# microsoft/StemGNN

Hardware: AMD Instinct MI355X
Metric: forecast-steps/sec (train) (higher is better)
Workload: dtype f32

## Files before the change

### include/stemgnn_hip.h

```cpp
#ifndef STEMGNN_HIP_H
#define STEMGNN_HIP_H

#include <stddef.h>
#include <stdint.h>

#ifdef __cplusplus
extern "C" {
#endif

#define SG_EINVAL (-10001)

#define SG_BLOCK_NPARAMS 33

const char* stemgnn_version(void);
int stemgnn_num_cus(void);

size_t stemgnn_table_floats(int W, int multi);
size_t stemgnn_packed_floats(int W, int multi);
size_t stemgnn_saved_floats(int B, int N, int W, int multi);
size_t stemgnn_scratch_floats(int B, int N, int W, int multi);
size_t stemgnn_gradpart_floats(int W, int multi, int nsplit);
size_t stemgnn_attn_saved_floats(int B, int N);
size_t stemgnn_attn_scratch_floats(int B, int N, int nchunk);
size_t stemgnn_scratch_offset_dG(int B, int N, int W, int multi);

int stemgnn_make_tables_host(int W, int multi, float* tables_host);

int stemgnn_attn_laplacian_fwd(const float* h, const float* wk, const float* wq, float alpha,
                               float drop_p, int training, const uint64_t* seed,
                               int B, int N, float* saved, float* attention_out, float* mul_L,
                               int parts, void* stream);
int stemgnn_attn_laplacian_bwd(const float* dL, const float* h, const float* wk, const float* wq,
                               float alpha, float drop_p, int training, const uint64_t* seed,
                               int B, int N, const float* saved, float* scratch, int nchunk,
                               float* dh, float* dwk, float* dwq, int parts, void* stream);
int stemgnn_attn_laplacian_bwd_ext(const float* dL, const float* dA_ext, const float* h, const float* wk, const float* wq,
                                   float alpha, float drop_p, int training, const uint64_t* seed,
                                   int B, int N, const float* saved, float* scratch, int nchunk,
                                   float* dh, float* dwk, float* dwq, int parts, void* stream);
int stemgnn_dropout_mask(float drop_p, const uint64_t* seed, int B, int N, float* mask, void* stream);
int stemgnn_dropout_seed_next(uint64_t* seed, uint64_t* used, void* stream);

int stemgnn_cheb_fwd(float* mul_L, int N, void* stream);
int stemgnn_cheb_bwd(const float* mul_L, const float* dmul_L, float* dL, float* scratch, int N, void* stream);

size_t stemgnn_eigh_scratch_floats(int N);
int stemgnn_eigh_fwd(float* mul_L, float* lam, float* U, float* scratch, int N, int nsweeps, void* stream);
int stemgnn_eigh_batched(float* mul_L, float* lam, float* U, float* scratch, int N, int batch, void* stream);
int stemgnn_eigh_status(void);
int stemgnn_eigh_cluster_fixes(void);

size_t stemgnn_split_planes_floats(int N, int K, int splits);
int stemgnn_split_weights_bf16(const float* B, int N, int K, int splits, void* planes, void* stream);
int stemgnn_glu_gemm_bf16(const float* A, const void* planes, float* C, int M, int N, int K, int splits, void* stream);
int stemgnn_glu_gemm_f32(const float* A, const float* B, float* C, int M, int N, int K, void* stream);

int stemgnn_sgemm_f32(const float* A, int lda, int a_kcontig, const float* B, int ldb, int b_kcontig, float* C, int ldc,
                      int M, int N, int K, int accumulate, void* stream);
int stemgnn_glu_combine_fwd(const float* U, const float* V, const float* bl, const float* br, float* out, float* gate,
                            float* lin, int M, int C, void* stream);
int stemgnn_glu_combine_bwd(const float* dout, const float* lin, const float* gate, float* dU, float* dV, int M, int C,
                            void* stream);
int stemgnn_colsum(const float* X, int M, int C, float* out, void* stream);

size_t stemgnn_gru_reserve_floats(int B, int S, int Hd);
size_t stemgnn_gru_fwd_scratch_floats(int B, int S, int Hd);
size_t stemgnn_gru_bwd_scratch_floats(int B, int S, int Hd, int W);
int stemgnn_gru_bwd_cus(int B, int Hd);
#define SG_GRU_PATH_WORDS 16
#define SG_GRU_FWD_FAMILY   0
#define SG_GRU_FWD_P        1
#define SG_GRU_FWD_K        2
#define SG_GRU_GI_STREAM    3
#define SG_GRU_BWD_FAMILY   4
#define SG_GRU_BWD_P        5
#define SG_GRU_BWD_KU       6
#define SG_GRU_BWD_SLICES   7
#define SG_GRU_IH_FOLDED    8
#define SG_GRU_HH_FORM      9
#define SG_GRU_IH_SLABS     10
#define SG_GRU_RANK2_OK     11
#define SG_GRU_WIDE_PASSES  12
#define SG_GRU_WIDE_MT      13
#define SG_GRU_WIDE_GWF     14
#define SG_GRU_WIDE_GWB     15
#define SG_GRU_FAM_STREAM   0
#define SG_GRU_FAM_CLUSTER1 1
#define SG_GRU_FAM_CLUSTER2 2
#define SG_GRU_FAM_CLUSTER4 3
#define SG_GRU_FAM_WIDE     4
#define SG_GRU_HH_SLABS     0
#define SG_GRU_HH_TILES     1
#define SG_GRU_HH_FLAT      2
int stemgnn_gru_paths(int B, int S, int Hd, int W, int cus, int* out );
int stemgnn_gru_fwd(const float* x, const float* w_ih, const float* w_hh, const float* b_ih, const float* b_hh,
                    int B, int S, int Hd, int W, float* scratch, float* h_ext, float* reserve, int* status,
                    void* stream);
int stemgnn_gru_bwd(const float* dh_all, const float* x, const float* w_hh, const float* h_ext,
                    const float* reserve, int B, int S, int Hd, int W, float* scratch,
                    float* dw_ih, float* dw_hh, float* db_ih, float* db_hh, int* status, void* stream);

int stemgnn_keyquery_wgrad(const float* h, const float* attn_scratch, float* dwk, float* dwq, int B, int N, void* stream);
int stemgnn_attn_dquery_reduce(float* attn_scratch, int B, int N, int nchunk, float* out, void* stream);
int stemgnn_keyquery_wgrad2(const float* h, const float* dkey, const float* dquery, float* dwk, float* dwq, int B, int N,
                            void* stream);
int stemgnn_gru_bwd_rank2_ok(int B, int Hd);
int stemgnn_gru_bwd_rank2(const float* dkey, const float* dquery, const float* wk, const float* wq, const float* x,
                          const float* w_hh, const float* h_ext, const float* reserve, int B, int S, int Hd, int W,
                          float* scratch, float* dw_ih, float* dw_hh, float* db_ih, float* db_hh, int* status, void* stream);
int stemgnn_gru_bwd_rank2_dq(const float* dkey, float* dquery, int nchunk, int flags, const float* wk, const float* wq, const float* x,
                             const float* w_hh, const float* h_ext, const float* reserve, int B, int S, int Hd, int W,
                             float* scratch, float* dw_ih, float* dw_hh, float* db_ih, float* db_hh, int* status, void* stream);
int stemgnn_gru_bwd_overlap_ok(int B, int S, int Hd, int W);
size_t stemgnn_gru_bwd_ctl_words(int S);
int stemgnn_gru_bwd_rank2_begin(const float* dkey, const float* dquery, const float* wk, const float* wq, const float* x,
                                const float* w_hh, const float* h_ext, const float* reserve, int B, int S, int Hd, int W,
                                float* scratch, float* dw_ih, float* dw_hh, float* db_ih, float* db_hh, int* status,
                                unsigned* ctl, void* stream);
int stemgnn_gru_bwd_rank2_finish(const float* dkey, const float* dquery, const float* wk, const float* wq, const float* x,
                                 const float* w_hh, const float* h_ext, const float* reserve, int B, int S, int Hd, int W,
                                 float* scratch, float* dw_ih, float* dw_hh, float* db_ih, float* db_hh, int* status,
                                 unsigned* ctl, void* side_stream, void* stream);
int stemgnn_gru_bwd_recur(const float* dh_all, const float* x, const float* w_hh, const float* h_ext, const float* reserve,
                          int B, int S, int Hd, int W, float* scratch, int* status, void* stream);
int stemgnn_gru_bwd_rank2_recur(const float* dkey, float* dquery, int nchunk, const float* wk, const float* wq, const float* x,
                                const float* w_hh, const float* h_ext, const float* reserve, int B, int S, int Hd, int W,
                                float* scratch, int* status, void* stream);
int stemgnn_gru_input_grad(const float* scratch, const float* w_ih, int B, int S, int Hd, int W, float* dx, void* stream);

int stemgnn_block_pack(const float* const* params_host, const float* tables, float* packed,
                       int W, int multi, void* stream);
int stemgnn_block_pack_panels(const float* const* params_host, const float* tables, float* packed, int W, int multi,
                              void* stream);
int stemgnn_glu_fused_repack(float* packed, int W, int multi, void* stream);
int stemgnn_block_unpack_grads(const float* gradpart, int nsplit, const float* tables,
                               float* const* grads_host, int W, int multi, int has_backcast, void* stream);

int stemgnn_gft_fwd(const float* mul_L, const float* X, long xs_b, long xs_n, long xs_t,
                    float* G, int B, int N, int W, void* stream);
int stemgnn_gft_bwd(const float* mul_L, const float* X, long xs_b, long xs_n, long xs_t,
                    const float* dG, float* dX, float* dmul_L, int accumulate,
                    int B, int N, int W, void* stream);
int stemgnn_gft_bwd_dt2(const float* X0, long xs0_b, long xs0_n, long xs0_t, const float* dG0, const float* X1, long xs1_b,
                        long xs1_n, long xs1_t, const float* dG1, float* dmul_L, int B, int N, int W, void* stream);

int stemgnn_spectral_glu_fwd(const float* packed, float* saved, int B, int N, int W, int multi, void* stream);
int stemgnn_spectral_glu_bwd(const float* packed, const float* saved, float* scratch, float* gradpart,
                             int nsplit, int parts, int B, int N, int W, int multi, void* stream);
size_t stemgnn_glu_split_floats(int W, int multi, int splits);
int stemgnn_glu_split_panels(const float* packed, float* split, int W, int multi, int splits, void* stream);
int stemgnn_spectral_glu_fwd_split(const float* packed, const float* split, float* saved, int B, int N, int W, int multi,
                                   int splits, void* stream);
size_t stemgnn_glu_warm_saved_floats(int W, int multi);
int stemgnn_spectral_glu_fwd_warm(const float* packed, const float* split, float* saved, int B, int N, int W, int multi,
                                  int splits, void* stream);
int stemgnn_spectral_glu_dgrad_split(const float* packed, const float* split, const float* saved, float* scratch,
                                     int B, int N, int W, int multi, int splits, void* stream);
int stemgnn_glu_fused_bf16_ok(int W, int multi, int splits);

int stemgnn_igft_heads_fwd(const float* const* params_host, const float* packed, float* saved,
                           const float* X, long xs_b, long xs_n, long xs_t,
                           float* forecast, int accumulate, float* backcast,
                           int B, int N, int W, int multi, void* stream);
int stemgnn_igft_heads_bwd(const float* const* params_host, const float* packed, const float* saved,
                           const float* X, long xs_b, long xs_n, long xs_t,
                           const float* dforecast, const float* dbackcast, const float* backcast,
                           float* scratch, float* gradpart, int nsplit, int parts,
                           int B, int N, int W, int multi, void* stream);

int stemgnn_shortcut_dx(const float* scratch, const float* bs_w, float* dX, int B, int N, int W, int multi, void* stream);

int stemgnn_block_wgrad(const float* const* params_host, const float* packed, const float* saved,
                        const float* X, long xs_b, long xs_n, long xs_t, const float* dforecast, int has_bc,
                        float* scratch, float* gradpart, int nsplit, int cu_percent,
                        int B, int N, int W, int multi, void* stream);
int stemgnn_block_wgrad_split(const float* const* params_host, const float* packed, const float* saved,
                              const float* X, long xs_b, long xs_n, long xs_t, const float* dforecast, int has_bc,
                              float* scratch, float* gradpart, int nsplit, int cu_percent, int B, int N, int W,
                              int multi, int splits, void* stream);

#define SG_PATH_GLU_FWD_FUSED   1
#define SG_PATH_GLU_DGRAD_FUSED 2
#define SG_PATH_HEADS_FWD_FUSED 4
#define SG_PATH_HEADS_BWD_FUSED 8
#define SG_PATH_HEADS_BWD_16W   16
#define SG_PATH_LONG_K          32
#define SG_PATH_WGRAD_FUSED     64
#define SG_PATH_GLU_WGRAD_FUSED 128
int stemgnn_block_paths(int B, int N, int W, int multi, int splits);

size_t stemgnn_infer_workspace_floats(int B, int N, int W, int multi);
size_t stemgnn_infer_workspace_split_floats(int B, int N, int W, int multi, int splits);
int stemgnn_gru_fwd_infer(const float* x, const float* w_ih, const float* w_hh, const float* b_ih, const float* b_hh,
                          int B, int S, int Hd, int W, float* scratch, float* h_ext, int* status, void* stream);
int stemgnn_spectral_glu_fwd_infer(const float* packed, float* ws, size_t ws_floats, int B, int N, int W, int multi,
                                   void* stream);
int stemgnn_spectral_glu_fwd_split_infer(const float* packed, const float* split, float* ws, size_t ws_floats, int B, int N,
                                         int W, int multi, int splits, void* stream);
int stemgnn_igft_heads_fwd_infer(const float* const* params_host, const float* packed, float* ws, size_t ws_floats,
                                 const float* X, long xs_b, long xs_n, long xs_t, float* forecast, int accumulate,
                                 float* backcast, int B, int N, int W, int multi, void* stream);

int stemgnn_fc_tail_supported(int W, int H);
size_t stemgnn_fc_tail_scratch_floats(int B, int N, int W, int H);
int stemgnn_fc_tail_fwd(const float* fsum, const float* w0, const float* b0, const float* w2, const float* b2,
                        int B, int N, int W, int H, float* forecast, void* stream);
int stemgnn_fc_tail_bwd(const float* dforecast, const float* fsum, const float* w0, const float* b0, const float* w2,
                        int B, int N, int W, int H, float* scratch, float* dfsum, float* dw0, float* db0,
                        float* dw2, float* db2, void* stream);
size_t stemgnn_fc_tail_train_scratch_floats(int B, int N, int W, int H);
int stemgnn_fc_tail_train(const float* fsum, const float* target, const float* w0, const float* b0, const float* w2,
                          const float* b2, int B, int N, int W, int H, float* scratch, float* forecast,
                          float* loss, double* loss_accum, float* dfsum, float* dw0, float* db0, float* dw2,
                          float* db2, void* stream);
int stemgnn_fc_tail_train_rows(const float* fsum, const float* target, const float* w0, const float* b0, const float* w2,
                               const float* b2, int B, int N, int W, int H, float* scratch, float* forecast, float* dfsum,
                               void* stream);
// ... 63 lines not shown
```

### stemgnn_amd/_lib.py

```python
import ctypes
import os
from ctypes import POINTER, c_char_p, c_float, c_int, c_long, c_size_t, c_void_p

_HERE = os.path.dirname(os.path.abspath(__file__))
LIB_PATH = os.environ.get("STEMGNN_HIP_LIB", os.path.join(_HERE, "libstemgnn_hip.so"))
SG_BLOCK_NPARAMS = 33
SG_EINVAL = -10001
SG_LOSS = {"mse": 0, "mae": 1, "huber": 2}
SG_PATH = {"glu_fwd_fused": 1, "glu_dgrad_fused": 2, "heads_fwd_fused": 4, "heads_bwd_fused": 8, "heads_bwd_16w": 16,
           "long_k": 32, "wgrad_fused": 64, "glu_wgrad_fused": 128}
SG_GRU_PATH_WORDS = 16
SG_GRU_WORD = {"fwd_family": 0, "fwd_P": 1, "fwd_K": 2, "gi_stream": 3, "bwd_family": 4, "bwd_P": 5, "bwd_KU": 6,
               "bwd_slices": 7, "ih_folded": 8, "hh_form": 9, "ih_slabs": 10, "rank2_ok": 11, "wide_passes": 12,
               "wide_MT": 13, "wide_GWf": 14, "wide_GWb": 15}
SG_GRU_FAM = {"stream": 0, "cluster1": 1, "cluster2": 2, "cluster4": 3, "wide": 4}
SG_GRU_HH = {"slabs": 0, "tiles": 1, "flat": 2}


def gru_paths(B, S, Hd, W, cus=0):
    out = (c_int * SG_GRU_PATH_WORDS)()
    check(load().stemgnn_gru_paths(B, S, Hd, W, cus, out), "stemgnn_gru_paths")
    return {k: int(out[i]) for k, i in SG_GRU_WORD.items()}


_P = c_void_p
_PP = POINTER(c_void_p)

SIGNATURES = {
    "stemgnn_version": (c_char_p, []),
    "stemgnn_num_cus": (c_int, []),
    "stemgnn_table_floats": (c_size_t, [c_int, c_int]),
    "stemgnn_packed_floats": (c_size_t, [c_int, c_int]),
    "stemgnn_saved_floats": (c_size_t, [c_int, c_int, c_int, c_int]),
    "stemgnn_scratch_floats": (c_size_t, [c_int, c_int, c_int, c_int]),
    "stemgnn_scratch_offset_dG": (c_size_t, [c_int, c_int, c_int, c_int]),
    "stemgnn_gradpart_floats": (c_size_t, [c_int, c_int, c_int]),
    "stemgnn_attn_saved_floats": (c_size_t, [c_int, c_int]),
    "stemgnn_attn_scratch_floats": (c_size_t, [c_int, c_int, c_int]),
    "stemgnn_make_tables_host": (c_int, [c_int, c_int, _P]),
    "stemgnn_attn_laplacian_fwd": (c_int, [_P, _P, _P, c_float, c_float, c_int, _P, c_int, c_int, _P, _P, _P, c_int, _P]),
    "stemgnn_attn_laplacian_bwd": (c_int, [_P, _P, _P, _P, c_float, c_float, c_int, _P, c_int, c_int, _P, _P, c_int,
                                           _P, _P, _P, c_int, _P]),
    "stemgnn_attn_laplacian_bwd_ext": (c_int, [_P, _P, _P, _P, _P, c_float, c_float, c_int, _P, c_int, c_int, _P, _P, c_int,
                                               _P, _P, _P, c_int, _P]),
    "stemgnn_dropout_mask": (c_int, [c_float, _P, c_int, c_int, _P, _P]),
    "stemgnn_dropout_seed_next": (c_int, [_P, _P, _P]),
    "stemgnn_cheb_fwd": (c_int, [_P, c_int, _P]),
    "stemgnn_cheb_bwd": (c_int, [_P, _P, _P, _P, c_int, _P]),
    "stemgnn_eigh_scratch_floats": (c_size_t, [c_int]),
    "stemgnn_eigh_fwd": (c_int, [_P, _P, _P, _P, c_int, c_int, _P]),
    "stemgnn_eigh_batched": (c_int, [_P, _P, _P, _P, c_int, c_int, _P]),
    "stemgnn_eigh_status": (c_int, []),
    "stemgnn_eigh_cluster_fixes": (c_int, []),
    "stemgnn_split_planes_floats": (c_size_t, [c_int, c_int, c_int]),
    "stemgnn_split_weights_bf16": (c_int, [_P, c_int, c_int, c_int, _P, _P]),
    "stemgnn_glu_gemm_bf16": (c_int, [_P, _P, _P, c_int, c_int, c_int, c_int, _P]),
    "stemgnn_glu_gemm_f32": (c_int, [_P, _P, _P, c_int, c_int, c_int, _P]),
    "stemgnn_sgemm_f32": (c_int, [_P, c_int, c_int, _P, c_int, c_int, _P, c_int, c_int, c_int, c_int, c_int, _P]),
    "stemgnn_glu_combine_fwd": (c_int, [_P, _P, _P, _P, _P, _P, _P, c_int, c_int, _P]),
    "stemgnn_glu_combine_bwd": (c_int, [_P, _P, _P, _P, _P, c_int, c_int, _P]),
    "stemgnn_colsum": (c_int, [_P, c_int, c_int, _P, _P]),
    "stemgnn_glu_fused_repack": (c_int, [_P, c_int, c_int, _P]),
    "stemgnn_shortcut_dx": (c_int, [_P, _P, _P, c_int, c_int, c_int, c_int, _P]),
    "stemgnn_gru_reserve_floats": (c_size_t, [c_int, c_int, c_int]),
    "stemgnn_gru_fwd_scratch_floats": (c_size_t, [c_int, c_int, c_int]),
    "stemgnn_gru_bwd_scratch_floats": (c_size_t, [c_int, c_int, c_int, c_int]),
    "stemgnn_gru_bwd_cus": (c_int, [c_int, c_int]),
    "stemgnn_gru_paths": (c_int, [c_int, c_int, c_int, c_int, c_int, POINTER(c_int)]),
    "stemgnn_gru_fwd": (c_int, [_P, _P, _P, _P, _P, c_int, c_int, c_int, c_int, _P, _P, _P, _P, _P]),
    "stemgnn_gru_bwd": (c_int, [_P, _P, _P, _P, _P, c_int, c_int, c_int, c_int, _P, _P, _P, _P, _P, _P, _P]),
    "stemgnn_gru_bwd_rank2_ok": (c_int, [c_int, c_int]),
    "stemgnn_gru_bwd_rank2": (c_int, [_P, _P, _P, _P, _P, _P, _P, _P, c_int, c_int, c_int, c_int, _P, _P, _P, _P, _P, _P, _P]),
    "stemgnn_gru_bwd_rank2_dq": (c_int, [_P, _P, c_int, c_int, _P, _P, _P, _P, _P, _P, c_int, c_int, c_int, c_int, _P, _P, _P, _P, _P, _P, _P]),
    "stemgnn_gru_bwd_overlap_ok": (c_int, [c_int, c_int, c_int, c_int]),
    "stemgnn_gru_bwd_ctl_words": (c_size_t, [c_int]),
    "stemgnn_gru_bwd_rank2_begin": (c_int, [_P, _P, _P, _P, _P, _P, _P, _P, c_int, c_int, c_int, c_int, _P, _P, _P, _P, _P, _P, _P, _P]),
    "stemgnn_gru_bwd_rank2_finish": (c_int, [_P, _P, _P, _P, _P, _P, _P, _P, c_int, c_int, c_int, c_int, _P, _P, _P, _P, _P, _P, _P, _P, _P]),
    "stemgnn_gru_bwd_recur": (c_int, [_P, _P, _P, _P, _P, c_int, c_int, c_int, c_int, _P, _P, _P]),
    "stemgnn_gru_bwd_rank2_recur": (c_int, [_P, _P, c_int, _P, _P, _P, _P, _P, _P, c_int, c_int, c_int, c_int, _P, _P, _P]),
    "stemgnn_gru_input_grad": (c_int, [_P, _P, c_int, c_int, c_int, c_int, _P, _P]),
    "stemgnn_keyquery_wgrad": (c_int, [_P, _P, _P, _P, c_int, c_int, _P]),
    "stemgnn_attn_dquery_reduce": (c_int, [_P, c_int, c_int, c_int, _P, _P]),
    "stemgnn_keyquery_wgrad2": (c_int, [_P, _P, _P, _P, _P, c_int, c_int, _P]),
    "stemgnn_fc_tail_supported": (c_int, [c_int, c_int]),
    "stemgnn_fc_tail_scratch_floats": (c_size_t, [c_int, c_int, c_int, c_int]),
    "stemgnn_fc_tail_fwd": (c_int, [_P, _P, _P, _P, _P, c_int, c_int, c_int, c_int, _P, _P]),
    "stemgnn_fc_tail_bwd": (c_int, [_P, _P, _P, _P, _P, c_int, c_int, c_int, c_int, _P, _P, _P, _P, _P, _P, _P]),
    "stemgnn_fill_zero": (c_int, [_P, c_size_t, _P]),
    "stemgnn_rmsprop_step": (c_int, [_P, _P, _P, c_size_t, _P, c_float, c_float, c_int, c_float, _P]),
    "stemgnn_adam_step": (c_int, [_P, _P, _P, _P, c_size_t, _P, _P, c_float, c_float, c_float, c_int, c_float, _P]),
    "stemgnn_grad_norm_partials": (c_size_t, [c_size_t]),
    "stemgnn_grad_sqsum": (c_int, [_P, c_size_t, c_float, _P, _P]),
    "stemgnn_rmsprop_step_ext": (c_int, [_P, _P, _P, c_size_t, _P, c_float, c_float, c_int, c_float, c_float, c_float, c_int,
                                         _P, _P, _P]),
    "stemgnn_adam_step_ext": (c_int, [_P, _P, _P, _P, c_size_t, _P, _P, c_float, c_float, c_float, c_int, c_float, c_float,
                                      c_int, c_float, c_int, _P, _P, _P]),
    "stemgnn_normalize_series": (c_int, [_P, _P, _P, c_int, _P, c_long, c_int, _P]),
    "stemgnn_window_gather": (c_int, [_P, _P, _P, _P, c_int, c_int, c_int, c_int, c_long, _P, _P]),
    "stemgnn_window_gather_queue": (c_int, [_P, _P, _P, _P, _P, c_int, c_int, c_int, c_int, c_long, _P, _P]),
    "stemgnn_window_gather_pair": (c_int, [_P, _P, _P, _P, _P, c_int, c_int, c_int, c_int, c_long, _P, _P]),
    "stemgnn_window_gather_queue_pair": (c_int, [_P, _P, _P, _P, _P, _P, c_int, c_int, c_int, c_int, c_long, _P, _P]),
    "stemgnn_mse_scratch_floats": (c_size_t, []),
    "stemgnn_mse_fwd": (c_int, [_P, _P, c_size_t, _P, _P, _P, _P]),
    "stemgnn_mse_bwd": (c_int, [_P, _P, c_size_t, _P, _P, _P]),
    "stemgnn_roll_window": (c_int, [_P, _P, _P, _P, c_int, c_int, c_int, c_int, c_int, c_int, _P]),
    "stemgnn_forecast_store": (c_int, [_P, _P, _P, _P, _P, c_int, c_int, c_int, c_long, _P]),
    "stemgnn_eval_scratch_doubles": (c_size_t, [c_long, c_int, c_int]),
    "stemgnn_eval_out_doubles": (c_size_t, [c_int, c_int]),
    "stemgnn_eval_metrics": (c_int, [_P, _P, _P, _P, c_long, c_int, c_int, _P, _P, _P]),
    "stemgnn_eval_scratch_doubles_masked": (c_size_t, [c_long, c_int, c_int]),
    "stemgnn_eval_metrics_masked": (c_int, [_P, _P, _P, _P, c_long, c_int, c_int, _P, _P, _P]),
    "stemgnn_block_pack": (c_int, [_PP, _P, _P, c_int, c_int, _P]),
    "stemgnn_block_pack_panels": (c_int, [_PP, _P, _P, c_int, c_int, _P]),
    "stemgnn_block_unpack_grads": (c_int, [_P, c_int, _P, _PP, c_int, c_int, c_int, _P]),
    "stemgnn_gft_fwd": (c_int, [_P, _P, c_long, c_long, c_long, _P, c_int, c_int, c_int, _P]),
    "stemgnn_gft_bwd": (c_int, [_P, _P, c_long, c_long, c_long, _P, _P, _P, c_int, c_int, c_int, c_int, _P]),
    "stemgnn_gft_bwd_dt2": (c_int, [_P, c_long, c_long, c_long, _P, _P, c_long, c_long, c_long, _P, _P, c_int, c_int, c_int, _P]),
    "stemgnn_spectral_glu_fwd": (c_int, [_P, _P, c_int, c_int, c_int, c_int, _P]),
    "stemgnn_spectral_glu_bwd": (c_int, [_P, _P, _P, _P, c_int, c_int, c_int, c_int, c_int, c_int, _P]),
    "stemgnn_glu_split_floats": (c_size_t, [c_int, c_int, c_int]),
    "stemgnn_glu_split_panels": (c_int, [_P, _P, c_int, c_int, c_int, _P]),
    "stemgnn_glu_fused_bf16_ok": (c_int, [c_int, c_int, c_int]),
    "stemgnn_block_paths": (c_int, [c_int, c_int, c_int, c_int, c_int]),
    "stemgnn_spectral_glu_fwd_split": (c_int, [_P, _P, _P, c_int, c_int, c_int, c_int, c_int, _P]),
    "stemgnn_glu_warm_saved_floats": (c_size_t, [c_int, c_int]),
    "stemgnn_spectral_glu_fwd_warm": (c_int, [_P, _P, _P, c_int, c_int, c_int, c_int, c_int, _P]),
    "stemgnn_spectral_glu_dgrad_split": (c_int, [_P, _P, _P, _P, c_int, c_int, c_int, c_int, c_int, _P]),
    "stemgnn_igft_heads_fwd": (c_int, [_PP, _P, _P, _P, c_long, c_long, c_long, _P, c_int, _P,
                                       c_int, c_int, c_int, c_int, _P]),
    "stemgnn_igft_heads_bwd": (c_int, [_PP, _P, _P, _P, c_long, c_long, c_long, _P, _P, _P, _P, _P, c_int, c_int,
                                       c_int, c_int, c_int, c_int, _P]),
    "stemgnn_fc_tail_train_scratch_floats": (c_size_t, [c_int, c_int, c_int, c_int]),
    "stemgnn_fc_tail_train": (c_int, [_P, _P, _P, _P, _P, _P, c_int, c_int, c_int, c_int, _P, _P, _P, _P, _P, _P, _P, _P,
                                      _P, _P]),
    "stemgnn_fc_tail_train_rows": (c_int, [_P, _P, _P, _P, _P, _P, c_int, c_int, c_int, c_int, _P, _P, _P, _P]),
    "stemgnn_fc_tail_train_finish": (c_int, [_P, c_int, c_int, c_int, c_int, _P, _P, _P, _P, _P, _P, _P]),
    "stemgnn_target_valid_count": (c_int, [_P, c_size_t, _P, _P]),
    "stemgnn_fc_tail_train_loss": (c_int, [_P, _P, _P, _P, _P, _P, c_int, c_int, c_int, c_int, c_int, c_float, _P, _P, _P, _P,
                                           _P, _P, _P, _P, _P, _P, _P]),
    "stemgnn_fc_tail_train_rows_loss": (c_int, [_P, _P, _P, _P, _P, _P, c_int, c_int, c_int, c_int, c_int, c_float, _P, _P, _P,
                                                _P, _P]),
    "stemgnn_fc_tail_train_finish_loss": (c_int, [_P, c_int, c_int, c_int, c_int, _P, _P, _P, _P, _P, _P, _P, _P]),
    "stemgnn_infer_workspace_floats": (c_size_t, [c_int, c_int, c_int, c_int]),
    "stemgnn_infer_workspace_split_floats": (c_size_t, [c_int, c_int, c_int, c_int, c_int]),
    "stemgnn_gru_fwd_infer": (c_int, [_P, _P, _P, _P, _P, c_int, c_int, c_int, c_int, _P, _P, _P, _P]),
    "stemgnn_spectral_glu_fwd_infer": (c_int, [_P, _P, c_size_t, c_int, c_int, c_int, c_int, _P]),
    "stemgnn_spectral_glu_fwd_split_infer": (c_int, [_P, _P, _P, c_size_t, c_int, c_int, c_int, c_int, c_int, _P]),
    "stemgnn_igft_heads_fwd_infer": (c_int, [_PP, _P, _P, c_size_t, _P, c_long, c_long, c_long, _P, c_int, _P,
                                             c_int, c_int, c_int, c_int, _P]),
    "stemgnn_block_wgrad": (c_int, [_PP, _P, _P, _P, c_long, c_long, c_long, _P, c_int, _P, _P, c_int, c_int,
                                    c_int, c_int, c_int, c_int, _P]),
    "stemgnn_block_wgrad_split": (c_int, [_PP, _P, _P, _P, c_long, c_long, c_long, _P, c_int, _P, _P, c_int, c_int,
                                          c_int, c_int, c_int, c_int, c_int, _P]),
}

_lib = None


class StemGNNHipError(RuntimeError):
    pass


def load():
    global _lib
    if _lib is not None:
        return _lib
    if not os.path.isfile(LIB_PATH):
        raise StemGNNHipError(
            f"{LIB_PATH} not found -- build it with `python __graft_entry__.py` (hipcc --offload-arch=gfx950); "
            "stemgnn_amd has no CPU / eager fallback.")
    lib = ctypes.CDLL(LIB_PATH)
    for name, (res, args) in SIGNATURES.items():
        fn = getattr(lib, name)
        fn.restype = res
        fn.argtypes = args
    _lib = lib
    return lib


def check(rc, what):
    if rc != 0:
        if rc == SG_EINVAL:
            raise StemGNNHipError(f"{what}: invalid argument (SG_EINVAL)")
        raise StemGNNHipError(f"{what}: HIP error {-rc}")


def ptr_array(tensors):
    arr = (c_void_p * SG_BLOCK_NPARAMS)()
    for i, t in enumerate(tensors):
        arr[i] = None if t is None else t.data_ptr()
    return arr
```

### stemgnn_amd/base_model.py

```python
import itertools
import os

import torch
import torch.nn as nn

from . import _lib, ops
from .ops import FcTail, FcTailMse, GruFront, SpectralHotPath, StockBlockFn

_instance_counter = itertools.count()
_BLOCK_FIELDS = ("forecast", "forecast_result", "backcast", "backcast_short_cut")
_FC_TAIL_MAX_W, _FC_TAIL_MAX_H = 64, 32


class GLU(nn.Module):

    def __init__(self, input_channel, output_channel):
        super().__init__()
        self.linear_left = nn.Linear(input_channel, output_channel)
        self.linear_right = nn.Linear(input_channel, output_channel)

    def forward(self, x):
        if not x.is_cuda:
            raise _lib.StemGNNHipError(f"input is on {x.device}: stemgnn_amd.GLU runs only on a HIP device (no CPU fallback)")
        lead = x.shape[:-1]
        out = ops.GluFn.apply(x.reshape(-1, x.shape[-1]), self.linear_left.weight, self.linear_left.bias,
                              self.linear_right.weight, self.linear_right.bias)
        return out.reshape(*lead, out.shape[-1])


class StockBlockLayer(nn.Module):

    def __init__(self, time_step, unit, multi_layer, stack_cnt=0):
        super().__init__()
        self.time_step, self.unit, self.multi, self.stack_cnt = time_step, unit, multi_layer, stack_cnt
        wide = time_step * multi_layer
        self.weight = nn.Parameter(torch.empty(1, 4, 1, wide, wide))
        nn.init.xavier_normal_(self.weight)
        self.forecast = nn.Linear(wide, wide)
        self.forecast_result = nn.Linear(wide, time_step)
        if stack_cnt == 0:
            self.backcast = nn.Linear(wide, time_step)
        self.backcast_short_cut = nn.Linear(time_step, time_step)
        self.output_channel = 4 * multi_layer
        glu_out = time_step * self.output_channel
        self.GLUs = nn.ModuleList(
            GLU(time_step * 4 if layer == 0 else glu_out, glu_out) for layer in range(3) for _branch in range(2))

    def hip_params(self):
        out = [self.weight]
        for name in _BLOCK_FIELDS:
            lin = getattr(self, name, None)
            out += [None, None] if lin is None else [lin.weight, lin.bias]
        for g in self.GLUs:
            out += [g.linear_left.weight, g.linear_left.bias, g.linear_right.weight, g.linear_right.bias]
        return out

    def forward(self, x, mul_L):
        if not x.is_cuda:
            raise _lib.StemGNNHipError(
                f"input is on {x.device}: stemgnn_amd.StockBlockLayer runs only on a HIP device (no CPU fallback)")
        B, _, N, W = x.shape
        forecast, backcast = StockBlockFn.apply(x.reshape(B, N, W), mul_L, self.multi, self.stack_cnt == 0,
                                                *self.hip_params())
        return forecast, (backcast.unsqueeze(1) if backcast is not None else None)


class Model(nn.Module):
    def __init__(self, units, stack_cnt, time_step, multi_layer, horizon=1, dropout_rate=0.5, leaky_rate=0.2,
                 device='cpu'):
        super().__init__()
        self.unit, self.stack_cnt, self.alpha = units, stack_cnt, leaky_rate
        self.time_step, self.horizon, self.multi_layer = time_step, horizon, multi_layer
        if time_step > _FC_TAIL_MAX_W or horizon > _FC_TAIL_MAX_H:
            raise _lib.StemGNNHipError(
                f"Model(time_step={time_step}, horizon={horizon}): the fc tail kernels (csrc/tail.hip) cover time_step <= "
                f"{_FC_TAIL_MAX_W} and horizon <= {_FC_TAIL_MAX_H}; stemgnn_amd has no torch fallback for larger ones")
        self.dropout_rate = float(dropout_rate)
        self.weight_key = nn.Parameter(torch.zeros(units, 1))
        nn.init.xavier_uniform_(self.weight_key.data, gain=1.414)
        self.weight_query = nn.Parameter(torch.zeros(units, 1))
        nn.init.xavier_uniform_(self.weight_query.data, gain=1.414)
        self.GRU = nn.GRU(time_step, units)
        self.stock_block = nn.ModuleList(
            StockBlockLayer(time_step, units, multi_layer, stack_cnt=i) for i in range(stack_cnt))
        self.fc = nn.Sequential(nn.Linear(time_step, time_step), nn.LeakyReLU(), nn.Linear(time_step, horizon))
        self._seed = None
        self._instance = next(_instance_counter)
        self.hot_state = ops.HotPathState()
        self.to(device)

    def _next_seed(self, device):
        if self._seed is None or self._seed.device != device:
            rank = 0
            if torch.distributed.is_available() and torch.distributed.is_initialized():
                rank = torch.distributed.get_rank()
            key = (torch.cuda.default_generators[device.index if device.index is not None
                                                 else torch.cuda.current_device()].initial_seed()
                   + 0x9E3779B97F4A7C15 * (self._instance + 1) + 0xD1B54A32D192ED03 * rank) % (1 << 62)
            self._seed = torch.tensor([key, 0], dtype=torch.int64, device=device)
        used = torch.empty_like(self._seed)
        _lib.check(_lib.load().stemgnn_dropout_seed_next(self._seed.data_ptr(), used.data_ptr(),
                                                         torch.cuda.current_stream(device).cuda_stream), "dropout_seed_next")
        return used

    def set_dropout_seed(self, seed, offset=0, device=None):
        device = device or self.weight_key.device
        self._seed = torch.tensor([int(seed), int(offset)], dtype=torch.int64, device=device)

    def __getstate__(self):
        state = self.__dict__.copy()
        state["_seed"] = None
        state["hot_state"] = None
        return state

    def __setstate__(self, state):
        self.__dict__.update(state)
        self._instance = next(_instance_counter)
        self.hot_state = ops.HotPathState()

    def train(self, mode=True):
        out = super().train(mode)
        dev = self.weight_key.device if hasattr(self, "weight_key") else None
        if dev is not None and dev.type == "cuda" and ops.gru_status_exists(dev) \
                and not torch.cuda.is_current_stream_capturing():
            ops.check_gru_status(dev)
            if os.environ.get("STEMGNN_SPECTRAL", "cheb") == "eig":
                ops.check_eigh_status(dev)
        return out

    def prefetch_side(self, device=None, batch=None):
        hs = self.hot_state
        if not hs.overlap or hs.prepacked is not None:
            return
        device = device or self.weight_key.device
        blocks = (self.stock_block[0].hip_params(), self.stock_block[1].hip_params())
        ops.prepack_blocks(hs, blocks, self.time_step, self.multi_layer, device,
                           batch_shape=None if batch is None else (int(batch), self.unit))
        if self.training and self.dropout_rate > 0.0:
            with torch.cuda.stream(ops._side_stream(device)):
                hs.preseed = self._next_seed(device)

    def hot_path(self, x):
        if not x.is_cuda:
            raise _lib.StemGNNHipError(
                f"input is on {x.device}: stemgnn_amd.Model runs only on a HIP device (no CPU fallback)")
        if self.stack_cnt > 2:
            raise AttributeError("'NoneType' object has no attribute 'unsqueeze'")
        if self.stack_cnt < 2:
            raise IndexError("list index out of range")
        x = x.contiguous()
        blocks = (self.stock_block[0].hip_params(), self.stock_block[1].hip_params())
        use_drop = self.training and self.dropout_rate > 0.0
        hs = self.hot_state
        if hs.overlap and hs.prepacked is None:
            self.prefetch_side(x.device, batch=x.shape[0])
        seed, hs.preseed = hs.preseed, None
        if seed is not None and not torch.cuda.is_current_stream_capturing():
            seed.record_stream(torch.cuda.current_stream())
        if os.environ.get("STEMGNN_GRU", "hip") == "miopen":
            h, _ = self.GRU(x.permute(2, 0, 1).contiguous())
        else:
            g = self.GRU
            h = GruFront.apply(x, g.weight_ih_l0, g.weight_hh_l0, g.bias_ih_l0, g.bias_hh_l0, hs)
            hs.gru_front_live = True
        if use_drop and seed is None:
            seed = self._next_seed(x.device)
        params = blocks[0] + blocks[1]
        return SpectralHotPath.apply(h, x, self.weight_key, self.weight_query, self.multi_layer, self.alpha,
                                     self.dropout_rate, self.training, seed, hs, *params)

    def loss(self, x, target, loss_out=None, accum=None, unit_grad=False, return_attention=False, *, kind="mse",
             huber_delta=1.0, ignore_nan=False):
        if kind not in _lib.SG_LOSS:
            raise ValueError(f"unknown loss kind {kind!r}: one of {sorted(_lib.SG_LOSS)}")
        self._require_fc_tail()
        fsum, attention, _ = self.hot_path(x)
        loss = FcTailMse.apply(fsum, target, self.fc[0].weight, self.fc[0].bias, self.fc[2].weight, self.fc[2].bias,
                               self.hot_state, loss_out, accum, bool(unit_grad) and torch.is_grad_enabled(), kind,
                               float(huber_delta) if kind == "huber" else 0.0, bool(ignore_nan))
        return (loss, attention) if return_attention else loss

    def _require_fc_tail(self):
        if not _lib.load().stemgnn_fc_tail_supported(self.time_step, self.horizon):
            raise _lib.StemGNNHipError(f"fc tail: time_step={self.time_step}, horizon={self.horizon} outside the HIP kernels' "
                                       "range (time_step <= 64, horizon <= 32); stemgnn_amd has no torch fallback")

    def predict(self, x):
        self._require_fc_tail()
        if not x.is_cuda:
            raise _lib.StemGNNHipError(
                f"input is on {x.device}: stemgnn_amd.Model runs only on a HIP device (no CPU fallback)")
        if self.stack_cnt > 2:
            raise AttributeError("'NoneType' object has no attribute 'unsqueeze'")
        if self.stack_cnt < 2:
            raise IndexError("list index out of range")
        g = self.GRU
        blocks = self.stock_block[0].hip_params() + self.stock_block[1].hip_params()
        with torch.no_grad():
            return ops.forecast_forward(x, (g.weight_ih_l0, g.weight_hh_l0, g.bias_ih_l0, g.bias_hh_l0), self.weight_key,
                                        self.weight_query, self.multi_layer, self.alpha, self.dropout_rate, blocks,
                                        (self.fc[0].weight, self.fc[0].bias, self.fc[2].weight, self.fc[2].bias))

    def forward(self, x):
        self._require_fc_tail()
        fsum, attention, _ = self.hot_path(x)
        return FcTail.apply(fsum, self.fc[0].weight, self.fc[0].bias, self.fc[2].weight, self.fc[2].bias,
                            self.hot_state), attention
```

### stemgnn_amd/csrc/glu_fused.h

```cpp
#pragma once
#include <hip/hip_runtime.h>
#include <stdint.h>

#include <type_traits>

#include "gemm2.h"
#include "layout.h"

constexpr int GF_NI = 4;
#ifndef GF_PF
#define GF_PF 2
#endif
#ifndef GF_ABL
#define GF_ABL 0
#endif

__device__ __forceinline__ float gf_sigmoid(float v) { return __frcp_rn(1.f + __expf(-v)); }
#ifndef GF_NT_STORES
#define GF_NT_STORES 1
#endif
#if GF_NT_STORES
#define GF_ST(p, v) __builtin_nontemporal_store((v), (p))
#else
#define GF_ST(p, v) (*(p) = (v))
#endif

struct GfPackArgs {
  const float* wp[2][3];
  float* wf[2];
  int K[3], np[2][3], cp[2][3];
  GfGeom g;
};
static __global__ __launch_bounds__(256) void sg_pack_fused_kernel(const GfPackArgs a) {
  const int r = blockIdx.y;
  const size_t e = (size_t)blockIdx.x * 256 + threadIdx.x;
  if (e >= (size_t)a.g.ns * GF_STAGE) return;
  int s = (int)(e / GF_STAGE), l = 0;
  while (l < 2 && s >= a.g.nst[l]) { s -= a.g.nst[l]; ++l; }
  const int hp = 16 / a.g.rs[l], nc = 256 * hp;
  const int w = (int)(e % GF_STAGE);
  const int kk = w / nc, p = w % nc;
  const int wave = p / (64 * hp), rem = p % (64 * hp), h = rem >> 6, fi = (rem & 63) >> 1, t = rem & 1;
  const int c = wave * 32 * hp + h * 32 + fi, k = s * a.g.rs[l] + kk;
  float v = 0.f;
  if (k < a.K[l] && c < a.cp[r][l]) v = a.wp[r][l][(size_t)k * a.np[r][l] + ((c >> 4) << 5) + (c & 15) + 16 * t];
  a.wf[r][e] = v;
}

struct GfArgs {
  const float* G;
  const float* wf[2];
  const float* bias[2][3];
  float* out[2][3];
  float* gate[2][3];
  int cp[2][3];
  int nst[3];
  int KG, KP0, KA, M, nrb, ns;
};

template <int N>
__device__ __forceinline__ void gf_wait_vm() { asm volatile("s_waitcnt vmcnt(%0)" ::"n"(N) : "memory"); }

struct GfRing {
  const float* src;
  float* ring;
  int next, last, wbuf, wave, nstages;
  __device__ __forceinline__ void issue(int q) {
    __builtin_amdgcn_global_load_lds((const __attribute__((address_space(1))) void*)(src + q * 256),
                                     (__attribute__((address_space(3))) void*)(ring + wbuf * GF_STAGE + (wave * GF_NI + q) * 256),
                                     16, 0, 0);
  }
  __device__ __forceinline__ void advance() {
    if (next < last) src += GF_STAGE;
    ++next;
    wbuf = wbuf + 1 == nstages ? 0 : wbuf + 1;
  }
};

template <int MT>
struct GfTile {
  static constexpr int BM = 32 * MT, LDA = 32 * MT + 2;
  static constexpr int STAGES = MT == 3 ? 4 : 5;
  static __device__ __forceinline__ int row(int i, int reg, int lane) {
    return i < 2 ? 2 * g2_row_of(reg, lane) + i : 64 + g2_row_of(reg, lane);
  }
};
template <int MT, int HP>
__device__ __forceinline__ void gf_stage(const float* __restrict__ Aq, const float* __restrict__ A2,
                                         const float* __restrict__ Bs, sg_f32x16 (&acc)[MT][HP][2], GfRing& rg) {
  constexpr int NC = 256 * HP, RS = 16 / HP, STEPS = RS / 2, LDA = GfTile<MT>::LDA;
  constexpr int EVERY = STEPS / GF_NI;
  float2 fa[STEPS], fb[STEPS][HP];
  float fc[STEPS];
  auto rd = [&](int st) {
    fa[st] = *reinterpret_cast<const float2*>(Aq + 2 * st * LDA);
    if constexpr (MT == 3) fc[st] = A2[2 * st * LDA];
#pragma unroll
    for (int h = 0; h < HP; ++h) fb[st][h] = *reinterpret_cast<const float2*>(Bs + 2 * st * NC + h * 64);
  };
#pragma unroll
  for (int st = 0; st < GF_PF && st < STEPS; ++st) rd(st);
#pragma unroll
  for (int st = 0; st < STEPS; ++st) {
    float a[3];
    a[0] = fa[st].x; a[1] = fa[st].y; a[2] = MT == 3 ? fc[st] : 0.f;
    __builtin_amdgcn_sched_barrier(0);
    if (!(GF_ABL & 2)) acc[0][0][0] = __builtin_amdgcn_mfma_f32_32x32x2f32(a[0], fb[st][0].x, acc[0][0][0], 0, 0, 0);
    if (st + GF_PF < STEPS) rd(st + GF_PF);
    __builtin_amdgcn_sched_barrier(0);
    if (!(GF_ABL & 2)) acc[0][0][1] = __builtin_amdgcn_mfma_f32_32x32x2f32(a[0], fb[st][0].y, acc[0][0][1], 0, 0, 0);
    if (!(GF_ABL & 4) && st % EVERY == 0 && st / EVERY < GF_NI) rg.issue(st / EVERY);
    __builtin_amdgcn_sched_barrier(0);
    if (!(GF_ABL & 2)) {
#pragma unroll
      for (int i = 0; i < MT; ++i)
#pragma unroll
        for (int h = 0; h < HP; ++h) {
          if (i == 0 && h == 0) continue;
          acc[i][h][0] = __builtin_amdgcn_mfma_f32_32x32x2f32(a[i], fb[st][h].x, acc[i][h][0], 0, 0, 0);
          acc[i][h][1] = __builtin_amdgcn_mfma_f32_32x32x2f32(a[i], fb[st][h].y, acc[i][h][1], 0, 0, 0);
        }
    }
  }
}

template <int MT, int HP, bool LAST, bool INF = false>
__device__ __forceinline__ void gf_layer(float* As, GfRing& rg, int& rbuf, int nst, int lane, int wave,
                                         const float (&bl)[2], const float (&br)[2], float* __restrict__ outp,
                                         float* __restrict__ gatep, int cp, int M, int m0, int KA) {
// ... 63 lines not shown
              GF_ST(&po[(size_t)rl * cp], o[reg][i]);
              if constexpr (!INF) GF_ST(&pg[(size_t)rl * cp], gs[reg][i]);
            }
          }
      }
    }
  }
  if constexpr (!LAST) asm volatile("s_waitcnt lgkmcnt(0)" ::: "memory");
  if (GF_ABL & 1) {
    if (acc[0][0][0][0] + acc[MT - 1][HP - 1][1][7] == 1.2345e-30f) As[0] = 1.f;
  }
}

template <int MT, int HP01, int HP2, bool INF = false>
static __global__ __launch_bounds__(256, 1) void sg_glu_fused_fwd_kernel(const GfArgs g) {
  using T = GfTile<MT>;
  extern __shared__ __attribute__((aligned(16))) float gf_lds[];
  float* As = gf_lds;
  const int L = blockIdx.x, xcd = L & 7;
  const int r = (xcd >> 2) & 1, rb = (L >> 3) * 4 + (xcd & 3);
  if (rb >= g.nrb) return;
  const int tid = threadIdx.x, lane = tid & 63;
  const int wave = __builtin_amdgcn_readfirstlane(tid >> 6);
  const int fi = lane & 31;
  const int m0 = rb * T::BM, M = g.M;

  GfRing rg;
  rg.ring = gf_lds + (size_t)g.KA * T::LDA;
  rg.wave = wave;
  rg.nstages = T::STAGES;
  rg.src = g.wf[r] + (size_t)wave * GF_NI * 256 + lane * 4;
  rg.next = 0; rg.last = g.ns - 1; rg.wbuf = 0;
#pragma unroll
  for (int p = 0; p < T::STAGES - 1; ++p) {
#pragma unroll
    for (int q = 0; q < GF_NI; ++q) rg.issue(q);
    rg.advance();
  }
  float bl[3][2], br[3][2];
#pragma unroll
  for (int l = 0; l < 3; ++l) {
    const int hp = l < 2 ? HP01 : HP2;
#pragma unroll
    for (int h = 0; h < 2; ++h) {
      const int c = wave * 32 * hp + h * 32 + fi;
      const bool ok = h < hp && c < g.cp[r][l];
      const int q = ((c >> 4) << 5) + (c & 15);
      const float* b = g.bias[r][l];
      const float x = b[ok ? q : 0], y = b[ok ? q + 16 : 0];
      bl[l][h] = ok ? x : 0.f;
      br[l][h] = ok ? y : 0.f;
    }
  }
  {
    const int KG = g.KG;
    const float* Gp = g.G + (size_t)m0 * KG;
    const int nlive = (M - m0 < T::BM ? M - m0 : T::BM) * KG;
    for (int idx = tid; idx < T::BM * KG; idx += 256) {
      const int i = idx / KG, k = idx - i * KG;
      const float v = Gp[idx < nlive ? idx : 0];
      As[k * T::LDA + i] = idx < nlive ? v : 0.f;
    }
    for (int idx = tid; idx < (g.KP0 - KG) * T::BM; idx += 256) As[(KG + idx / T::BM) * T::LDA + (idx % T::BM)] = 0.f;
  }
#pragma unroll
  for (int l = 0; l < 3; ++l)
#pragma unroll
    for (int h = 0; h < 2; ++h) asm volatile("" : "+v"(bl[l][h]), "+v"(br[l][h]));
  asm volatile("s_waitcnt lgkmcnt(0)" ::: "memory");
  int rbuf = 0;
  gf_layer<MT, HP01, false, INF>(As, rg, rbuf, g.nst[0], lane, wave, bl[0], br[0], g.out[r][0], g.gate[r][0], g.cp[r][0], M, m0, g.KA);
  gf_layer<MT, HP01, false, INF>(As, rg, rbuf, g.nst[1], lane, wave, bl[1], br[1], g.out[r][1], g.gate[r][1], g.cp[r][1], M, m0, g.KA);
  gf_layer<MT, HP2, true, INF>(As, rg, rbuf, g.nst[2], lane, wave, bl[2], br[2], g.out[r][2], g.gate[r][2], g.cp[r][2], M, m0, g.KA);
  gf_wait_vm<0>();
}

struct GdPackArgs {
  const float* wp[2][3];
  float* wd[2];
  int np[2][3];
  int CP, KG;
  GdGeom g;
};
static __global__ __launch_bounds__(256) void sg_pack_dgrad_kernel(const GdPackArgs a) {
  const int r = blockIdx.y;
  const size_t e = (size_t)blockIdx.x * 256 + threadIdx.x;
  if (e >= (size_t)a.g.ns[r] * GF_STAGE) return;
  int s = (int)(e / GF_STAGE);
  const int nt = a.g.nt, rs = a.g.rs, nc = 128 * nt;
  const int wi = (int)(e % GF_STAGE);
  const int sAB = a.g.nstA[r] + a.g.nstB[0] + a.g.nstB[1];
  if (s >= sAB) {
    s -= sAB;
    int ph = 0;
    if (s >= a.g.nstC[0]) { s -= a.g.nstC[0]; ph = 1; }
    const int kk = wi >> 6, kin = wi & 63;
    const int k2 = s * 64 + kk;
    const int t = k2 & 1, wf = k2 >> 1, w2 = wf >> 5, f2 = wf & 31;
    const int c2 = w2 * 32 * nt + 32 * ph + f2;
    float v = 0.f;
    if (w2 < 4 && c2 < a.CP && kin < a.KG) v = a.wp[r][0][(size_t)kin * a.np[r][0] + ((c2 >> 4) << 5) + (c2 & 15) + 16 * t];
    a.wd[r][e] = v;
    return;
  }
  const int kk = wi / nc, p = wi % nc;
  int wave, fi, j;
  if (nt == 2) { wave = p >> 6; fi = (p & 63) >> 1; j = p & 1; }
  else { wave = p >> 5; fi = p & 31; j = 0; }
  const int c = wave * 32 * nt + 32 * j + fi;
  float v = 0.f;
  if (s < a.g.nstA[r]) {
    const int q = s * rs + kk;
    if (q < a.np[r][2] && c < a.CP) v = a.wp[r][2][(size_t)c * a.np[r][2] + q];
  } else {
    s -= a.g.nstA[r];
    int ph = 0;
    if (s >= a.g.nstB[0]) { s -= a.g.nstB[0]; ph = 1; }
    const int k2 = s * rs + kk;
    const int t = k2 & 1, wf = k2 >> 1, w2 = wf >> 5, f2 = wf & 31;
    const int c2 = w2 * 32 * nt + 32 * ph + f2;
    if (w2 < 4 && c2 < a.CP && c < a.CP) v = a.wp[r][1][(size_t)c * a.np[r][1] + ((c2 >> 4) << 5) + (c2 & 15) + 16 * t];
  }
  a.wd[r][e] = v;
}

struct GdArgs {
  const float* dact2[2];
  const float* wd[2];
  const float* out1[2];
  const float* gate1[2];
  const float* out0[2];
  const float* gate0[2];
  float* dact1[2];
  float* dact0[2];
  float* dG[2];
  int np2[2], nstA[2], ns[2];
  int nstB[2], nstC[2];
  int CP, KG, M, nrb, KA;
};

template <int MT>
struct GdTile {
  static constexpr int BM = 32 * MT, LDA = 32 * MT + 2;
  static constexpr int STAGES = MT == 3 ? 3 : 5;
};

template <int MT, int NT>
__device__ __forceinline__ void gd_stage(const float* __restrict__ Aq, const float* __restrict__ A2,
                                         const float* __restrict__ Bs, sg_f32x16 (&acc)[MT][NT], GfRing& rg) {
  constexpr int NC = 128 * NT, RS = 32 / NT, STEPS = RS / 2, LDA = GdTile<MT>::LDA;
  constexpr int EVERY = STEPS / GF_NI;
  float2 fa[STEPS];
  float fc[STEPS];
  float fb[STEPS][2];
  auto rd = [&](int st) {
    fa[st] = *reinterpret_cast<const float2*>(Aq + 2 * st * LDA);
    if constexpr (MT == 3) fc[st] = A2[2 * st * LDA];
    if constexpr (NT == 2) {
      const float2 b = *reinterpret_cast<const float2*>(Bs + 2 * st * NC);
      fb[st][0] = b.x; fb[st][1] = b.y;
    } else {
      fb[st][0] = Bs[2 * st * NC]; fb[st][1] = 0.f;
    }
  };
#pragma unroll
  for (int st = 0; st < GF_PF && st < STEPS; ++st) rd(st);
#pragma unroll
  for (int st = 0; st < STEPS; ++st) {
    float a[3];
    a[0] = fa[st].x; a[1] = fa[st].y; a[2] = MT == 3 ? fc[st] : 0.f;
    __builtin_amdgcn_sched_barrier(0);
    if (!(GF_ABL & 2)) acc[0][0] = __builtin_amdgcn_mfma_f32_32x32x2f32(a[0], fb[st][0], acc[0][0], 0, 0, 0);
    if (st + GF_PF < STEPS) rd(st + GF_PF);
    __builtin_amdgcn_sched_barrier(0);
    if (!(GF_ABL & 2)) acc[1][0] = __builtin_amdgcn_mfma_f32_32x32x2f32(a[1], fb[st][0], acc[1][0], 0, 0, 0);
    if (!(GF_ABL & 4) && st % EVERY == 0 && st / EVERY < GF_NI) rg.issue(st / EVERY);
    __builtin_amdgcn_sched_barrier(0);
    if (!(GF_ABL & 2)) {
      if constexpr (MT == 3) acc[2][0] = __builtin_amdgcn_mfma_f32_32x32x2f32(a[2], fb[st][0], acc[2][0], 0, 0, 0);
      if constexpr (NT == 2) {
#pragma unroll
        for (int i = 0; i < MT; ++i) acc[i][1] = __builtin_amdgcn_mfma_f32_32x32x2f32(a[i], fb[st][1], acc[i][1], 0, 0, 0);
      }
    }
  }
}

template <int MT>
__device__ __forceinline__ void gd_stage_c(const float* __restrict__ Aq, const float* __restrict__ A2,
                                           const float* __restrict__ Bs, sg_f32x16& acc, sg_f32x16& acc2, bool extra,
                                           GfRing& rg) {
  constexpr int STEPS = 32, EVERY = STEPS / GF_NI, PF = 4, LDA = GdTile<MT>::LDA;
  float fa[STEPS], fb[STEPS], fc[STEPS];
  auto rd = [&](int st) {
    fa[st] = Aq[2 * st * LDA];
    fb[st] = Bs[2 * st * 64];
    if constexpr (MT == 3) fc[st] = A2[2 * st * LDA];
  };
#pragma unroll
  for (int st = 0; st < PF; ++st) rd(st);
#pragma unroll
  for (int st = 0; st < STEPS; ++st) {
    __builtin_amdgcn_sched_barrier(0);
    if (!(GF_ABL & 2)) acc = __builtin_amdgcn_mfma_f32_32x32x2f32(fa[st], fb[st], acc, 0, 0, 0);
    if constexpr (MT == 3) {
      if (extra && !(GF_ABL & 2)) acc2 = __builtin_amdgcn_mfma_f32_32x32x2f32(fc[st], fb[st], acc2, 0, 0, 0);
// ... 263 lines not shown
```

### stemgnn_amd/csrc/gru.hip

```cpp
#include <hip/hip_runtime.h>

#include "../../include/stemgnn_hip.h"
#include "gemm2.h"
#include "wgrad.h"
#include "dq_reduce.h"
#include "gemm_core.h"
#include "gru_wide.h"

#define SG_TRY(e)                                \
  do {                                           \
    hipError_t _e = (e);                         \
    if (_e != hipSuccess) return -(int)_e;       \
  } while (0)

__device__ __forceinline__ float gru_sigmoid(float v) { return 1.f / (1.f + expf(-v)); }
__device__ __forceinline__ int gru_uniform(int v) { return __builtin_amdgcn_readfirstlane(v); }

struct GruGiOp {
  const float *x, *w_ih, *b_ih;
  float* gi;
  int B, S, Hd, W;
  unsigned *za, *zb;
  unsigned na, nb;
  __device__ bool setup(int, int& M, int& N, int& K0, int& K1) const {
    M = S * B; N = 3 * Hd; K0 = 0; K1 = W;
    if (na + nb) {
      const unsigned nwg = gridDim.x * gridDim.y, id = blockIdx.y * gridDim.x + blockIdx.x;
      const unsigned per = (na + nb + nwg - 1) / nwg, hi = min(na + nb, (id + 1) * per);
      for (unsigned i = id * per + threadIdx.x; i < hi; i += blockDim.x) {
        if (i < na) za[i] = 0u;
        else zb[i - na] = 0u;
      }
    }
    return true;
  }
  __device__ float a(int, int i, int k) const {
    const int s = i / B, b = i - s * B;
    return x[((size_t)b * W + k) * S + s];
  }
  __device__ float b(int, int k, int j) const { return w_ih[(size_t)j * W + k]; }
  __device__ void epi(int, int i, int j, float v) const { gi[(size_t)i * 3 * Hd + j] = v + b_ih[j]; }
};

struct GruDxOp {
  const float *dgi, *w_ih;
  float* dx;
  int B, S, Hd, W;
  __device__ bool setup(int, int& M, int& N, int& K0, int& K1) const {
    M = S * B; N = W; K0 = 0; K1 = 3 * Hd;
    return true;
  }
  __device__ float a(int, int i, int k) const {
    const int b = i / S, s = i - b * S;
    return dgi[((size_t)s * B + b) * 3 * Hd + k];
  }
  __device__ float b(int, int k, int j) const { return w_ih[(size_t)k * W + j]; }
  __device__ void epi(int, int i, int j, float v) const {
    const int b = i / S, s = i - b * S;
    dx[((size_t)b * W + j) * S + s] = v;
  }
};

constexpr int GI_RB = 16, GI_NT = 192;
template <int W>
__global__ __launch_bounds__(GI_NT) void gru_gi_stream_kernel(const float* __restrict__ x, const float* __restrict__ w_ih,
                                                              const float* __restrict__ b_ih, float* __restrict__ gi, int B,
                                                              int S, int Hd, unsigned* __restrict__ za,
                                                              unsigned* __restrict__ zb, unsigned na, unsigned nb) {
  __shared__ float xs[GI_RB][W];
  const int tid = threadIdx.x;
  const int M = S * B, H3 = 3 * Hd, ncg = H3 >> 2;
  const int i0 = blockIdx.x * GI_RB;
  const int cg = blockIdx.y * GI_NT + tid;
  const bool live = cg < ncg;
  const int cgc = live ? cg : ncg - 1;
  float wf[4 * W];
  {
    const float* wp = w_ih + (size_t)4 * cgc * W;
    if ((reinterpret_cast<uintptr_t>(w_ih) & 15) == 0) {
#pragma unroll
      for (int q = 0; q < W; ++q) {
        const float4 v = reinterpret_cast<const float4*>(wp)[q];
        wf[4 * q] = v.x; wf[4 * q + 1] = v.y; wf[4 * q + 2] = v.z; wf[4 * q + 3] = v.w;
      }
    } else {
#pragma unroll
      for (int q = 0; q < 4 * W; ++q) wf[q] = wp[q];
    }
  }
  float4 bias;
  bias.x = b_ih[4 * cgc]; bias.y = b_ih[4 * cgc + 1]; bias.z = b_ih[4 * cgc + 2]; bias.w = b_ih[4 * cgc + 3];
  for (int e = tid; e < GI_RB * W; e += GI_NT) {
    const int r = e / W, k = e - r * W;
    const int i = i0 + r < M ? i0 + r : M - 1;
    const int sI = i / B, b = i - sI * B;
    xs[r][k] = x[((size_t)b * W + k) * S + sI];
  }
  if (na + nb) {
    const unsigned nwg = gridDim.x * gridDim.y, id = blockIdx.y * gridDim.x + blockIdx.x;
    const unsigned per = (na + nb + nwg - 1) / nwg, hi = min(na + nb, (id + 1) * per);
    for (unsigned i = id * per + tid; i < hi; i += GI_NT) {
      if (i < na) za[i] = 0u;
      else zb[i - na] = 0u;
    }
  }
  __syncthreads();
#pragma unroll 4
  for (int r = 0; r < GI_RB; ++r) {
    float a0 = 0.f, a1 = 0.f, a2 = 0.f, a3 = 0.f;
#pragma unroll
    for (int k = 0; k < W; ++k) {
      const float xv = xs[r][k];
      a0 = fmaf(xv, wf[k], a0);
      a1 = fmaf(xv, wf[W + k], a1);
      a2 = fmaf(xv, wf[2 * W + k], a2);
      a3 = fmaf(xv, wf[3 * W + k], a3);
    }
    if (live && i0 + r < M)
      *reinterpret_cast<float4*>(gi + (size_t)(i0 + r) * H3 + 4 * cg) = make_float4(a0 + bias.x, a1 + bias.y, a2 + bias.z, a3 + bias.w);
  }
}

__global__ void gru_transpose_kernel(const float* __restrict__ w, float* __restrict__ wT, int rows, int cols) {
  __shared__ float t[32][33];
  const int tx = threadIdx.x & 31, ty = threadIdx.x >> 5;
  const int r0 = blockIdx.y * 32, c0 = blockIdx.x * 32;
  for (int r = ty; r < 32; r += 8)
    t[r][tx] = (r0 + r < rows && c0 + tx < cols) ? w[(size_t)(r0 + r) * cols + c0 + tx] : 0.f;
  __syncthreads();
  for (int r = ty; r < 32; r += 8)
    if (c0 + r < cols && r0 + tx < rows) wT[(size_t)(c0 + r) * rows + r0 + tx] = t[tx][r];
}

template <bool RS>
__global__ __launch_bounds__(1024) void gru_fwd_kernel(const float* __restrict__ gi, const float* __restrict__ w_hhT,
                                                       const float* __restrict__ b_hh, int B, int S, int Hd,
                                                       float* __restrict__ h_all, float* __restrict__ reserve) {
  extern __shared__ __attribute__((aligned(16))) float smem[];
  float* hs = smem;
  float* part = smem + Hd;
  const int b = blockIdx.x;
  const int tid = threadIdx.x, lane = tid & 63, wave = tid >> 6;
  const int nub = (Hd + 63) >> 6;
  const int ks = nub >= 16 ? 1 : 16 / nub;
  const int kchunk = (Hd + ks - 1) / ks;
  const int nwork = nub * ks;
  const int H3 = 3 * Hd;
  for (int i = tid; i < Hd; i += 1024) hs[i] = 0.f;
  __syncthreads();
  for (int s = 0; s < S; ++s) {
    for (int item = wave; item < nwork; item += 16) {
      const int ub = item % nub, kq = item / nub;
      const int unit = ub * 64 + lane;
      const int uc = unit < Hd ? unit : Hd - 1;
      const int k0 = kq * kchunk, k1 = min(Hd, k0 + kchunk);
      float a0 = 0.f, a1 = 0.f, a2 = 0.f;
      const float* wp = w_hhT + (size_t)k0 * H3 + uc;
#pragma unroll 8
      for (int k = k0; k < k1; ++k) {
        const float hv = hs[k];
        a0 = fmaf(wp[0], hv, a0);
        a1 = fmaf(wp[Hd], hv, a1);
        a2 = fmaf(wp[2 * Hd], hv, a2);
        wp += H3;
      }
      if (unit < Hd) {
        part[(kq * 3 + 0) * Hd + unit] = a0;
        part[(kq * 3 + 1) * Hd + unit] = a1;
        part[(kq * 3 + 2) * Hd + unit] = a2;
      }
    }
    __syncthreads();
    const size_t row = (size_t)s * B + b;
    for (int i = tid; i < Hd; i += 1024) {
      float g0 = b_hh[i], g1 = b_hh[Hd + i], g2 = b_hh[2 * Hd + i];
      for (int q = 0; q < ks; ++q) {
        g0 += part[(q * 3 + 0) * Hd + i];
        g1 += part[(q * 3 + 1) * Hd + i];
        g2 += part[(q * 3 + 2) * Hd + i];
      }
      const float* gip = gi + row * H3;
      const float r = gru_sigmoid(gip[i] + g0);
      const float z = gru_sigmoid(gip[Hd + i] + g1);
      const float n = tanhf(gip[2 * Hd + i] + r * g2);
      const float hn = (1.f - z) * n + z * hs[i];
      if constexpr (RS) {
        float* rs = reserve + row * 4 * Hd;
        rs[i] = r; rs[Hd + i] = z; rs[2 * Hd + i] = n; rs[3 * Hd + i] = g2;
      }
      h_all[row * Hd + i] = hn;
      hs[i] = hn;
    }
    __syncthreads();
  }
}

__global__ __launch_bounds__(1024) void gru_bwd_kernel(const float* __restrict__ dout, const float* __restrict__ w_hh,
                                                       const float* __restrict__ h_all, const float* __restrict__ reserve,
                                                       int B, int S, int Hd, float* __restrict__ dgi,
                                                       float* __restrict__ dghn) {
  extern __shared__ __attribute__((aligned(16))) float smem[];
  float* dgh = smem;
  float* dhz = smem + 3 * Hd;
// ... 661 lines not shown
  const int smax_ws = (int)(ws_floats / ((size_t)f.ntiles * WG_TILE_FLOATS));
  if (smax_ws >= 1) { f.form = SG_GRU_HH_TILES; f.smax = smax_ws > 32 ? 32 : smax_ws; }
  return f;
}
struct GruPlan {
  int fwd_family, PF, KF, gi_stream;
  int bwd_family, P, KU, slices, fold_ih, hh_form, ih_sum, rank2_ok;
  GruWide wide;
};
static GruPlan gru_plan(int B, int S, int Hd, int W, int limit) {
  GruPlan p{};
  const int P2 = gru_pick_P2(B, Hd, limit);
  if (gru_pick_wide(B, Hd, P2, limit, &p.wide) > 0) {
    p.fwd_family = p.bwd_family = SG_GRU_FAM_WIDE;
  } else if (P2 > 0) {
    p.fwd_family = SG_GRU_FAM_CLUSTER4;
    p.PF = P2;
    {
      const int want = 7, uw = (Hd + want - 1) / want;
      if (uw <= 40 && B * want <= limit) p.PF = want;
    }
    const int UF = (Hd + p.PF - 1) / p.PF;
    p.KF = UF <= 32 ? 32 : (UF <= 34 ? 34 : (UF <= 40 ? 40 : (UF <= 48 ? 48 : (UF <= 58 ? 58 : 64))));
    const bool v4 = P2 <= 4 || P2 == 6;
    p.bwd_family = v4 ? SG_GRU_FAM_CLUSTER4 : SG_GRU_FAM_CLUSTER2;
    p.P = P2;
    p.KU = gru_pick_KU(Hd, P2);
    if (P2 == 6 && p.KU < 58) p.KU = 58;
    p.slices = (P2 == 6 || P2 == 8) ? 2 : 1;
    p.fold_ih = v4 && W <= GRU4_WMAX;
    p.rank2_ok = v4;
  } else {
    const int P = gru_pick_P(B, Hd, limit);
    p.fwd_family = p.bwd_family = P > 0 ? SG_GRU_FAM_CLUSTER1 : SG_GRU_FAM_STREAM;
    p.PF = p.P = P;
  }
  p.gi_stream = gru_gi_stream_env() && p.fwd_family != SG_GRU_FAM_WIDE && W == 12 && (Hd & 3) == 0;
  p.ih_sum = p.fold_ih ? B : GRU_NSPLIT;
  {
    float* const base = reinterpret_cast<float*>((uintptr_t)256);
    WgGemm q[2];
    gru_hh_gemms(q, base, base + (size_t)3 * S * B * Hd, base, base, base, Hd);
    p.hh_form = gru_hh_form(q, Hd).form;
  }
  return p;
}
extern "C" int stemgnn_gru_paths(int B, int S, int Hd, int W, int cus, int* out) {
  if (B <= 0 || S <= 0 || Hd <= 0 || W <= 0 || !out) return SG_EINVAL;
  const GruPlan p = gru_plan(B, S, Hd, W, cus > 0 ? gru_limit_of_cus(cus) : gru_resident_limit());
  const bool wide = p.fwd_family == SG_GRU_FAM_WIDE;
  out[SG_GRU_FWD_FAMILY] = p.fwd_family; out[SG_GRU_FWD_P] = p.PF; out[SG_GRU_FWD_K] = p.KF;
  out[SG_GRU_GI_STREAM] = p.gi_stream;
  out[SG_GRU_BWD_FAMILY] = p.bwd_family; out[SG_GRU_BWD_P] = p.P; out[SG_GRU_BWD_KU] = p.KU;
  out[SG_GRU_BWD_SLICES] = p.slices; out[SG_GRU_IH_FOLDED] = p.fold_ih; out[SG_GRU_HH_FORM] = p.hh_form;
  out[SG_GRU_IH_SLABS] = p.ih_sum; out[SG_GRU_RANK2_OK] = p.rank2_ok;
  out[SG_GRU_WIDE_PASSES] = wide ? (B + GW_BP - 1) / GW_BP : 0;
  out[SG_GRU_WIDE_MT] = wide ? p.wide.MT : 0;
  out[SG_GRU_WIDE_GWF] = wide ? gru_wide_gwf_class(p.wide) : 0;
  out[SG_GRU_WIDE_GWB] = wide ? gru_wide_gwb_class(p.wide) : 0;
  return 0;
}

extern "C" size_t stemgnn_gru_fwd_scratch_floats(int B, int S, int Hd) {
  return (size_t)3 * Hd * Hd + (size_t)3 * S * B * Hd + gru_xbuf_floats(B, Hd) + 4;
}
static size_t gru_bwd_scratch_base(int B, int S, int Hd, int W) {
  return (size_t)4 * S * B * Hd + (size_t)GRU_NSPLIT * 3 * Hd * (Hd + 1) + (size_t)gru_ih_slabs(B) * 3 * Hd * (W + 1) +
         gru_xbuf_floats(B, Hd) + 4 + (size_t)B * Hd + 8 + 136;
}
constexpr size_t GRU_OVL_CLAIMS = 64 * 33;
static size_t gru_ovl_words(int S) { return (((size_t)S + 4 + GRU_OVL_CLAIMS + 64 + 8) + 3) & ~(size_t)3; }
extern "C" size_t stemgnn_gru_bwd_scratch_floats(int B, int S, int Hd, int W) {
  return ((gru_bwd_scratch_base(B, S, Hd, W) + 3) & ~(size_t)3) + gru_ovl_words(S);
}
extern "C" size_t stemgnn_gru_bwd_ctl_words(int S) { return S > 0 ? gru_ovl_words(S) + 64 : 0; }

extern "C" int stemgnn_gru_bwd_cus(int B, int Hd) {
  if (B <= 0 || Hd <= 0) return 0;
  const GruPlan pl = gru_plan(B, Hd, Hd, 1, gru_resident_limit());
  if (pl.bwd_family == SG_GRU_FAM_WIDE) return pl.wide.P;
  return B * (pl.P > 0 ? pl.P : 1);
}

template <bool RS>
static int gru_fwd_impl(const float* x, const float* w_ih, const float* w_hh, const float* b_ih, const float* b_hh, int B,
                        int S, int Hd, int W, float* scratch, float* h_ext, float* reserve, int* status, void* stream) {
  if (!x || !w_ih || !w_hh || !b_ih || !b_hh || !scratch || !h_ext || (RS && !reserve) || !status || B <= 0 || S <= 0 ||
      Hd <= 0 || W <= 0)
    return SG_EINVAL;
  hipStream_t st = (hipStream_t)stream;
  const GruPlan pl = gru_plan(B, S, Hd, W, gru_resident_limit());
  const bool use_wide = pl.fwd_family == SG_GRU_FAM_WIDE, use_c4 = pl.fwd_family == SG_GRU_FAM_CLUSTER4;
  float* h_all = h_ext + (size_t)B * Hd;
  float* w_hhT = scratch;
  float* gi = scratch + (size_t)3 * Hd * Hd;
  gru_u64* xbuf2 = (gru_u64*)(scratch + ((((size_t)3 * Hd * Hd + (size_t)3 * S * B * Hd) + 1) & ~(size_t)1));
  size_t zn0 = 0, zn1 = 0;
  if (use_c4) {
    zn0 = (size_t)B * Hd; zn1 = ((size_t)2 * B * Hd + (size_t)8 * B) * 2;
  } else {
    SG_TRY(sg_zero_async(h_ext, (size_t)B * Hd * sizeof(float), st));
  }
  if (pl.gi_stream && (reinterpret_cast<uintptr_t>(gi) & 15) == 0) {
    const int ncg = 3 * Hd / 4;
    hipLaunchKernelGGL(gru_gi_stream_kernel<12>, dim3((S * B + GI_RB - 1) / GI_RB, (ncg + GI_NT - 1) / GI_NT), dim3(GI_NT), 0,
                       st, x, w_ih, b_ih, gi, B, S, Hd, reinterpret_cast<unsigned*>(h_ext), reinterpret_cast<unsigned*>(xbuf2),
                       (unsigned)zn0, (unsigned)zn1);
    SG_TRY(hipGetLastError());
  } else {
    GruGiOp op{x, w_ih, b_ih, gi, B, S, Hd, W, reinterpret_cast<unsigned*>(h_ext), reinterpret_cast<unsigned*>(xbuf2),
               (unsigned)zn0, (unsigned)zn1};
    SG_TRY((sg_launch_gemm<GruGiOp, 64, 64, true, true, false>(op, S * B, 3 * Hd, 1, st)));
  }
  if (use_wide) {
    float* xb = scratch + ((((size_t)3 * Hd * Hd + (size_t)3 * S * B * Hd) + 3) & ~(size_t)3);
    SG_TRY(gru_wide_fwd<RS>(gi, w_hh, b_hh, B, S, Hd, pl.wide, xb, status, h_all, reserve, st));
    return 0;
  }
  if (use_c4) {
    gru_u64* xbuf = xbuf2;
    gru_u64* xid = xbuf + (size_t)2 * B * Hd;
    static const int allow_fast = !(getenv("STEMGNN_GRU_FAST_XCD") && atoi(getenv("STEMGNN_GRU_FAST_XCD")) == 0);
    const int PF = pl.PF, KF = pl.KF;
    const dim3 grid4(8 * ((B + 7) / 8) * PF);
#define GRU_F4K(PP, KK) hipLaunchKernelGGL((gru_fwd_cluster4_kernel<PP, KK, RS>), grid4, dim3((PP + 2) * 64), 0, st, gi, w_hh, \
                                           b_hh, B, S, Hd, xbuf, status, h_all, reserve, xid, allow_fast)
#define GRU_F4(PP) do { if (KF == 32) GRU_F4K(PP, 32); else if (KF == 34) GRU_F4K(PP, 34); else if (KF == 40) GRU_F4K(PP, 40); \
                        else if (KF == 48) GRU_F4K(PP, 48); else if (KF == 58) GRU_F4K(PP, 58); else GRU_F4K(PP, 64); } while (0)
    if (PF == 1) GRU_F4(1); else if (PF == 2) GRU_F4(2); else if (PF == 4) GRU_F4(4); else if (PF == 5) GRU_F4(5);
    else if (PF == 6) GRU_F4(6); else if (PF == 7) GRU_F4(7); else GRU_F4(8);
#undef GRU_F4
#undef GRU_F4K
    SG_TRY(hipGetLastError());
    return 0;
  }
  if (pl.fwd_family == SG_GRU_FAM_CLUSTER1) {
    const int P = pl.PF;
    const GruCluster c = gru_cluster_geom(Hd, P);
    gru_u64* xbuf = (gru_u64*)(scratch + ((((size_t)3 * Hd * Hd + (size_t)3 * S * B * Hd) + 1) & ~(size_t)1));
    if (P > 1) SG_TRY(sg_zero_async(xbuf, (size_t)2 * B * Hd * sizeof(gru_u64), st));
    const size_t lds = (size_t)(Hd + GRU_KC + c.ksf * 3 * c.U) * sizeof(float);
    const dim3 grid(8 * ((B + 7) / 8) * P);
    hipLaunchKernelGGL((gru_fwd_cluster_kernel<GRU_KC, RS>), grid, dim3(1024), lds, st, gi, w_hh, b_hh, B, S, Hd, P, xbuf,
                       status, h_all, reserve);
    SG_TRY(hipGetLastError());
    return 0;
  }
  hipLaunchKernelGGL(gru_transpose_kernel, dim3((Hd + 31) / 32, (3 * Hd + 31) / 32), dim3(256), 0, st, w_hh, w_hhT,
                     3 * Hd, Hd);
  SG_TRY(hipGetLastError());
  const int nub = (Hd + 63) / 64;
  const int ks = nub >= 16 ? 1 : 16 / nub;
  const size_t lds = (size_t)(Hd + ks * 3 * Hd) * sizeof(float);
  if (lds > 64 * 1024) return SG_EINVAL;
  hipLaunchKernelGGL(gru_fwd_kernel<RS>, dim3(B), dim3(1024), lds, st, gi, w_hhT, b_hh, B, S, Hd, h_all, reserve);
  SG_TRY(hipGetLastError());
  return 0;
}

extern "C" int stemgnn_gru_fwd(const float* x, const float* w_ih, const float* w_hh, const float* b_ih,
                               const float* b_hh, int B, int S, int Hd, int W, float* scratch, float* h_ext,
                               float* reserve, int* status, void* stream) {
  return gru_fwd_impl<true>(x, w_ih, w_hh, b_ih, b_hh, B, S, Hd, W, scratch, h_ext, reserve, status, stream);
}
extern "C" int stemgnn_gru_fwd_infer(const float* x, const float* w_ih, const float* w_hh, const float* b_ih,
                                     const float* b_hh, int B, int S, int Hd, int W, float* scratch, float* h_ext,
                                     int* status, void* stream) {
  return gru_fwd_impl<false>(x, w_ih, w_hh, b_ih, b_hh, B, S, Hd, W, scratch, h_ext, nullptr, status, stream);
}

static int gru_wgrad_rows(const float* dgi, const float* dghn, const float* h_ext, const float* x, float* p_hh, float* p_ih,
                          int B, int S, int Hd, int W, int row0, int rows, int slab0, int nsplit, hipStream_t st_hh,
                          hipStream_t st_ih, bool do_ih = true, bool do_hh = true) {
  const int chunk = ((rows + nsplit - 1) / nsplit + 15) & ~15;
  if (do_hh) {
    G2Args g;
    G2SlabEpi e;
    g.A[0] = dgi + (size_t)row0 * 3 * Hd;  g.lda[0] = 3 * Hd; g.M[0] = 2 * Hd;
    g.A[1] = dghn + (size_t)row0 * Hd;     g.lda[1] = Hd;     g.M[1] = Hd;
    for (int r = 0; r < 2; ++r) { g.B[r] = h_ext + (size_t)row0 * Hd; g.ldb[r] = Hd; g.N[r] = Hd + 1; g.K[r] = rows; }
    g.nsplit = nsplit; g.chunk = chunk; g.b_ones_col = Hd;
    e.part[0] = p_hh + (size_t)slab0 * 2 * Hd * (Hd + 1);
    e.part[1] = p_hh + (size_t)GRU_NSPLIT * 2 * Hd * (Hd + 1) + (size_t)slab0 * Hd * (Hd + 1);
    SG_TRY((g2_launch<G2SlabEpi, false, false>(g, e, 2, st_hh)));
  }
  if (!do_ih) return 0;
  GruWihGradOp o2{dgi, x, p_ih + (size_t)slab0 * 3 * Hd * (W + 1), B, S, Hd, W, nsplit, chunk, row0, rows};
  SG_TRY((sg_launch_gemm<GruWihGradOp, 64, 32, false, false, false, 64>(o2, 3 * Hd, W + 1, nsplit, st_ih)));
  return 0;
}
extern "C" int stemgnn_gru_bwd_rank2_ok(int B, int Hd) {
  if (B <= 0 || Hd <= 0) return 0;
  return gru_plan(B, Hd, Hd, 1, gru_resident_limit()).rank2_ok;
}
static int gru_bwd_impl(const float* dh_all, const float* dkey, const float* dquery, const float* wk, const float* wq,
                        const float* x, const float* w_hh, const float* h_ext, const float* reserve, int B, int S, int Hd,
                        int W, float* scratch, float* dw_ih, float* dw_hh, float* db_ih, float* db_hh, int* status,
                        void* stream, int stages = 3, void* side = nullptr, unsigned* ctl = nullptr, int dq_nchunk = 0,
                        int wg_split = 0, bool no_wgrad = false);
extern "C" int stemgnn_gru_bwd(const float* dh_all, const float* x, const float* w_hh, const float* h_ext,
                               const float* reserve, int B, int S, int Hd, int W, float* scratch, float* dw_ih,
                               float* dw_hh, float* db_ih, float* db_hh, int* status, void* stream) {
  if (!dh_all) return SG_EINVAL;
  return gru_bwd_impl(dh_all, nullptr, nullptr, nullptr, nullptr, x, w_hh, h_ext, reserve, B, S, Hd, W, scratch, dw_ih, dw_hh,
                      db_ih, db_hh, status, stream);
}
extern "C" int stemgnn_gru_bwd_rank2(const float* dkey, const float* dquery, const float* wk, const float* wq, const float* x,
                                     const float* w_hh, const float* h_ext, const float* reserve, int B, int S, int Hd, int W,
                                     float* scratch, float* dw_ih, float* dw_hh, float* db_ih, float* db_hh, int* status,
                                     void* stream) {
  if (!dkey || !dquery || !wk || !wq || !stemgnn_gru_bwd_rank2_ok(B, Hd)) return SG_EINVAL;
  return gru_bwd_impl(nullptr, dkey, dquery, wk, wq, x, w_hh, h_ext, reserve, B, S, Hd, W, scratch, dw_ih, dw_hh, db_ih, db_hh,
                      status, stream);
}
__global__ __launch_bounds__(256) void sg_gru_fill_dq_kernel(uint32_t* __restrict__ p, size_t n16, unsigned nfill,
                                                             const float* __restrict__ dqpart, float* __restrict__ dquery, int B,
                                                             int N, int nchunk) {
  if (blockIdx.x < nfill) {
    uint4* q = reinterpret_cast<uint4*>(p);
    for (size_t k = (size_t)blockIdx.x * 256 + threadIdx.x; k < n16; k += (size_t)nfill * 256) q[k] = make_uint4(0u, 0u, 0u, 0u);
    return;
  }
  const size_t idx = (size_t)(blockIdx.x - nfill) * 256 + threadIdx.x;
  if (idx < (size_t)B * N) sg_dquery_reduce_one(dqpart, dquery, N, nchunk, idx);
}
__global__ void sg_gru_dq_reduce_kernel(const float* __restrict__ dqpart, float* __restrict__ dquery, int B, int N, int nchunk) {
  const size_t idx = (size_t)blockIdx.x * blockDim.x + threadIdx.x;
  if (idx < (size_t)B * N) sg_dquery_reduce_one(dqpart, dquery, N, nchunk, idx);
}
extern "C" int stemgnn_gru_bwd_rank2_dq(const float* dkey, float* dquery, int nchunk, int flags, const float* wk, const float* wq,
                                        const float* x, const float* w_hh, const float* h_ext, const float* reserve, int B, int S,
                                        int Hd, int W, float* scratch, float* dw_ih, float* dw_hh, float* db_ih, float* db_hh,
                                        int* status, void* stream) {
  if (!dkey || !dquery || nchunk <= 0 || (flags & ~1) || !wk || !wq || !stemgnn_gru_bwd_rank2_ok(B, Hd)) return SG_EINVAL;
  return gru_bwd_impl(nullptr, dkey, dquery, wk, wq, x, w_hh, h_ext, reserve, B, S, Hd, W, scratch, dw_ih, dw_hh, db_ih, db_hh,
                      status, stream, 3, nullptr, nullptr, nchunk, flags & 1);
}
extern "C" int stemgnn_gru_bwd_recur(const float* dh_all, const float* x, const float* w_hh, const float* h_ext,
                                     const float* reserve, int B, int S, int Hd, int W, float* scratch, int* status,
                                     void* stream) {
  if (!dh_all) return SG_EINVAL;
  return gru_bwd_impl(dh_all, nullptr, nullptr, nullptr, nullptr, x, w_hh, h_ext, reserve, B, S, Hd, W, scratch, nullptr, nullptr,
                      nullptr, nullptr, status, stream, 3, nullptr, nullptr, 0, 0, true);
}
extern "C" int stemgnn_gru_bwd_rank2_recur(const float* dkey, float* dquery, int nchunk, const float* wk, const float* wq,
                                           const float* x, const float* w_hh, const float* h_ext, const float* reserve, int B,
// ... 262 lines not shown
```

### stemgnn_amd/csrc/pack.hip

```cpp
#include <hip/hip_runtime.h>
#include <math.h>

#include "../../include/stemgnn_hip.h"
#include "devattr.h"
#include "glu_fused.h"
#include "layout.h"

#define SG_TRY(e)                                \
  do {                                           \
    hipError_t _e = (e);                         \
    if (_e != hipSuccess) return -(int)_e;       \
  } while (0)

struct SgBlockParams { const float* p[SG_BLOCK_NPARAMS]; };
struct SgBlockGrads { float* p[SG_BLOCK_NPARAMS]; };

__host__ __device__ inline int sg_pidx_glu(int g, int side, int bias) { return 9 + 4 * g + 2 * side + bias; }

static void exact_cos_sin(long idx, long n, double* c, double* s) {
  idx %= n;
  if ((4 * idx) % n == 0) {
    static const double cs[4] = {1, 0, -1, 0}, sn[4] = {0, 1, 0, -1};
    const long qd = 4 * idx / n;
    *c = cs[qd]; *s = sn[qd];
    return;
  }
  const double ang = 2.0 * M_PI * (double)idx / (double)n;
  *c = cos(ang); *s = sin(ang);
}

extern "C" int stemgnn_make_tables_host(int W, int multi, float* t) {
  if (W <= 0 || multi <= 0 || !t) return SG_EINVAL;
  const SgDims d = sg_dims(1, 1, W, multi);
  const SgTableLayout L = sg_table_layout(d);
  for (int tt = 0; tt < W; ++tt)
    for (int f = 0; f < W; ++f) {
      double c, s;
      exact_cos_sin((long)tt * f, W, &c, &s);
      t[L.cosW + tt * W + f] = (float)c;
      t[L.sinW + tt * W + f] = (float)s;
    }
  const int Wm = d.Wm, h = Wm / 2;
  for (int f = 0; f < d.nf[0]; ++f) {
    const double cf = (f == 0 || (Wm % 2 == 0 && f == h)) ? 1.0 : 2.0;
    for (int tau = 0; tau < Wm; ++tau) {
      double c, s;
      exact_cos_sin((long)f * tau, Wm, &c, &s);
      t[L.cinvR + (size_t)f * Wm + tau] = (float)(cf * c / Wm);
    }
  }
  for (int fi = 0; fi < d.nf[1]; ++fi) {
    const int f = fi + 1;
    for (int tau = 0; tau < Wm; ++tau) {
      double c, s;
      exact_cos_sin((long)f * tau, Wm, &c, &s);
      t[L.cinvI + (size_t)fi * Wm + tau] = (float)(-2.0 * s / Wm);
    }
  }
  return 0;
}

extern "C" const char* stemgnn_version(void) { return "stemgnn_hip 0.1 gfx950"; }
extern "C" int stemgnn_num_cus(void) { return sg_num_cus(); }
extern "C" size_t stemgnn_table_floats(int W, int multi) { return sg_table_layout(sg_dims(1, 1, W, multi)).total; }
extern "C" size_t stemgnn_packed_floats(int W, int multi) { return sg_packed_layout(sg_dims(1, 1, W, multi)).total_ext; }
extern "C" size_t stemgnn_saved_floats(int B, int N, int W, int multi) { return sg_saved_layout(sg_dims(B, N, W, multi)).total; }
extern "C" size_t stemgnn_scratch_floats(int B, int N, int W, int multi) { return sg_scratch_layout(sg_dims(B, N, W, multi)).total; }
extern "C" size_t stemgnn_scratch_offset_dG(int B, int N, int W, int multi) { return sg_scratch_layout(sg_dims(B, N, W, multi)).dG; }
extern "C" size_t stemgnn_gradpart_floats(int W, int multi, int nsplit) {
  return sg_grad_layout(sg_dims(1, 1, W, multi), nsplit).total;
}

__global__ void sg_pack_kernel(SgBlockParams prm, const float* __restrict__ tab, float* __restrict__ packed, SgDims d,
                               SgPackedLayout P, SgTableLayout T) {
  const size_t idx = (size_t)blockIdx.x * blockDim.x + threadIdx.x;
  if (idx >= P.total) return;
  const int W = d.W, Wm = d.Wm, C = d.C;
  float val = 0.f;
  if (idx >= P.wfold) {
    const size_t e = idx - P.wfold;
    const int kk = (int)(e / d.WmP), o = (int)(e - (size_t)kk * d.WmP);
    const int r = kk >= d.CP2[0];
    const int c = kk - (r ? d.CP2[0] : 0);
    if (c < d.U[r] && o < Wm) {
      const int kq = c / d.nf[r], fi = c - kq * d.nf[r];
      const float* cinv = tab + (r ? T.cinvI : T.cinvR) + (size_t)fi * Wm;
      const float* wt = prm.p[0] + (size_t)kq * Wm * Wm + o;
      float s0 = 0.f, s1 = 0.f, s2 = 0.f, s3 = 0.f;
      int tau = 0;
      for (; tau + 3 < Wm; tau += 4) {
        s0 = fmaf(cinv[tau], wt[(size_t)tau * Wm], s0);
        s1 = fmaf(cinv[tau + 1], wt[(size_t)(tau + 1) * Wm], s1);
        s2 = fmaf(cinv[tau + 2], wt[(size_t)(tau + 2) * Wm], s2);
        s3 = fmaf(cinv[tau + 3], wt[(size_t)(tau + 3) * Wm], s3);
      }
      for (; tau < Wm; ++tau) s0 = fmaf(cinv[tau], wt[(size_t)tau * Wm], s0);
      val = (s0 + s1) + (s2 + s3);
    }
    packed[idx] = val;
    return;
  }
  for (int r = 0; r < 2; ++r)
    for (int l = 0; l < 3; ++l) {
      const int np = sg_glu_np(d, l, r), kin = sg_glu_kin(d, l), cu = sg_glu_cu(d, l, r);
      const int g = 2 * l + r;
      if (idx >= P.w[r][l] && idx < P.w[r][l] + (size_t)kin * np) {
        const size_t e = idx - P.w[r][l];
        const int kk = (int)(e / np), q = (int)(e - (size_t)kk * np);
        const int c = ((q >> 5) << 4) + (q & 15), side = (q >> 4) & 1;
        if (c < cu) {
          const int ch = l < 2 ? c : sg_l2_orig_channel(d, r, c);
          const float* w = prm.p[sg_pidx_glu(g, side, 0)];
          if (l == 0) {
            const int kq = kk / W + 1, t = kk - (kq - 1) * W;
            const float* row = w + (size_t)ch * (4 * W) + kq * W;
            const float* dt = tab + (r ? T.sinW : T.cosW) + t * W;
            float s = 0.f;
            for (int f = 0; f < W; ++f) s = fmaf(dt[f], row[f], s);
            val = r ? -s : s;
          } else if (kk < C) {
            val = w[(size_t)ch * C + kk];
          }
        }
        packed[idx] = val;
        return;
      }
      if (idx >= P.b[r][l] && idx < P.b[r][l] + (size_t)np) {
        const int q = (int)(idx - P.b[r][l]);
        const int c = ((q >> 5) << 4) + (q & 15), side = (q >> 4) & 1;
        if (c < cu) {
          const int ch = l < 2 ? c : sg_l2_orig_channel(d, r, c);
          val = prm.p[sg_pidx_glu(g, side, 1)][ch];
        }
        packed[idx] = val;
        return;
      }
    }
}

extern "C" int stemgnn_block_pack_panels(const float* const* params_host, const float* tables, float* packed, int W,
                                         int multi, void* stream) {
  if (!params_host || !tables || !packed || W <= 0 || multi <= 0) return SG_EINVAL;
  SgBlockParams prm;
  for (int i = 0; i < SG_BLOCK_NPARAMS; ++i) prm.p[i] = params_host[i];
  for (int i = 0; i < SG_BLOCK_NPARAMS; ++i)
    if (!prm.p[i] && i != 5 && i != 6) return SG_EINVAL;
  const SgDims d = sg_dims(1, 1, W, multi);
  const SgPackedLayout P = sg_packed_layout(d);
  const SgTableLayout T = sg_table_layout(d);
  const unsigned blocks = (unsigned)((P.total + 255) / 256);
  hipLaunchKernelGGL(sg_pack_kernel, dim3(blocks), dim3(256), 0, (hipStream_t)stream, prm, tables, packed, d, P, T);
  SG_TRY(hipGetLastError());
  return 0;
}
extern "C" int stemgnn_block_pack(const float* const* params_host, const float* tables, float* packed, int W,
                                  int multi, void* stream) {
  const int rc = stemgnn_block_pack_panels(params_host, tables, packed, W, multi, stream);
  if (rc) return rc;
  return stemgnn_glu_fused_repack(packed, W, multi, stream);
}

extern "C" int stemgnn_glu_fused_repack(float* packed, int W, int multi, void* stream) {
  if (!packed || W <= 0 || multi <= 0) return SG_EINVAL;
  const SgDims d = sg_dims(1, 1, W, multi);
  const SgPackedLayout P = sg_packed_layout(d);
  const GfGeom gg = gf_geom(d);
  if (gg.ok) {
    GfPackArgs a;
    a.g = gg;
    for (int l = 0; l < 3; ++l) {
      a.K[l] = sg_glu_kin(d, l);
      for (int r = 0; r < 2; ++r) {
        a.wp[r][l] = packed + P.w[r][l];
        a.np[r][l] = sg_glu_np(d, l, r);
        a.cp[r][l] = sg_glu_cp(d, l, r);
      }
    }
    for (int r = 0; r < 2; ++r) a.wf[r] = packed + P.wfused[r];
    const unsigned fb = (unsigned)(((size_t)gg.ns * GF_STAGE + 255) / 256);
    hipLaunchKernelGGL(sg_pack_fused_kernel, dim3(fb, 2), dim3(256), 0, (hipStream_t)stream, a);
    SG_TRY(hipGetLastError());
  }
  const GdGeom gd = gd_geom(d);
  if (gd.ok) {
    GdPackArgs a;
    a.g = gd;
    a.CP = d.CP; a.KG = d.KG;
    for (int l = 0; l < 3; ++l)
      for (int r = 0; r < 2; ++r) {
        a.wp[r][l] = packed + P.w[r][l];
        a.np[r][l] = sg_glu_np(d, l, r);
      }
    for (int r = 0; r < 2; ++r) a.wd[r] = packed + P.wdgrad[r];
    const int nsmax = gd.ns[0] > gd.ns[1] ? gd.ns[0] : gd.ns[1];
    const unsigned fb = (unsigned)(((size_t)nsmax * GF_STAGE + 255) / 256);
    hipLaunchKernelGGL(sg_pack_dgrad_kernel, dim3(fb, 2), dim3(256), 0, (hipStream_t)stream, a);
    SG_TRY(hipGetLastError());
  }
  return 0;
}

struct SgParamOffsets { size_t prefix[SG_BLOCK_NPARAMS + 1]; };

__global__ void sg_unpack_kernel(const float* __restrict__ part, const float* __restrict__ tab, SgBlockGrads gr,
                                 SgParamOffsets PO, SgDims d, SgGradLayout G, SgTableLayout T, int has_bc) {
  const size_t idx = (size_t)blockIdx.x * blockDim.x + threadIdx.x;
  if (idx >= PO.prefix[SG_BLOCK_NPARAMS]) return;
  int pi = 0;
  while (pi + 1 < SG_BLOCK_NPARAMS && idx >= PO.prefix[pi + 1]) ++pi;
  float* out = gr.p[pi];
  if (!out) return;
  const size_t e = idx - PO.prefix[pi];
  const int W = d.W, Wm = d.Wm, C = d.C;
  float val = 0.f;
  if (pi == 0) {
    const int kq = (int)(e / ((size_t)Wm * Wm));
    const int rem = (int)(e - (size_t)kq * Wm * Wm);
    const int tau = rem / Wm, o = rem - tau * Wm;
    const float* wf = part + G.wfold;
    float s0 = 0.f, s1 = 0.f;
#pragma unroll 4
    for (int f = 0; f < d.nf[0]; ++f)
      s0 = fmaf(tab[T.cinvR + (size_t)f * Wm + tau], wf[(size_t)(kq * d.nf[0] + f) * d.WmP + o], s0);
#pragma unroll 4
    for (int f = 0; f < d.nf[1]; ++f)
      s1 = fmaf(tab[T.cinvI + (size_t)f * Wm + tau], wf[(size_t)(d.CP2[0] + kq * d.nf[1] + f) * d.WmP + o], s1);
    val = s0 + s1;
  } else if (pi <= 8) {
    const int isb = (pi - 1) & 1;
    const int which = (pi - 1) >> 1;
    if (which >= 2 && !has_bc) { out[e] = 0.f; return; }
    const float* p; int in;
    switch (which) {
      case 0: p = part + G.fc; in = Wm; break;
      case 1: p = part + G.fr; in = Wm; break;
      case 2: p = part + G.bc; in = Wm; break;
      default: p = part + G.bs; in = W; break;
    }
    if (isb) val = p[e * (in + 1) + in];
    else { const size_t o = e / in; val = p[o * (in + 1) + (e - o * in)]; }
  } else {
    const int gq = (pi - 9) >> 2, rem = (pi - 9) & 3, side = rem >> 1, isb = rem & 1;
    const int l = gq >> 1, r = gq & 1;
    const int kin = sg_glu_kin(d, l), cin = l == 0 ? 4 * W : C;
    const int ch = isb ? (int)e : (int)(e / cin);
    const int ki = isb ? 0 : (int)(e - (size_t)ch * cin);
    int c = ch;
    bool live = true;
    if (l == 2) {
      const int kq = ch / Wm, f = ch - kq * Wm;
      const int fi = f - (r ? 1 : 0);
      live = fi >= 0 && fi < d.nf[r];
      c = kq * d.nf[r] + fi;
    }
    if (live) {
      const int q = ((c >> 4) << 5) + (c & 15) + (side ? 16 : 0);
      const float* row = part + G.w[r][l] + (size_t)q * (kin + 1);
      if (isb) val = row[kin];
      else if (l == 0) {
        const int kq = ki / W, f = ki - kq * W;
        if (kq > 0) {
          const float* dt = tab + (r ? T.sinW : T.cosW);
          float s = 0.f;
          for (int t = 0; t < W; ++t) s = fmaf(dt[t * W + f], row[(kq - 1) * W + t], s);
          val = r ? -s : s;
        }
      } else {
        val = row[ki];
      }
    }
  }
  out[e] = val;
}

extern "C" int stemgnn_block_unpack_grads(const float* gradpart, int nsplit, const float* tables,
                                          float* const* grads_host, int W, int multi, int has_backcast,
                                          void* stream) {
  if (!gradpart || !tables || !grads_host || nsplit <= 0 || W <= 0 || multi <= 0) return SG_EINVAL;
  const SgDims d = sg_dims(1, 1, W, multi);
// ... 27 lines not shown
```

### stemgnn_amd/engine.py

```python
import os
import sys
import time

import torch

from . import _lib, ops
from .distributed import FlatGradBucket


def _active_collectives():
    try:
        import pickle
        from torch._C import _distributed_c10d as c10d
        dump = getattr(c10d, "_dump_nccl_trace", None)
        if dump is None:
            return None
        everything = pickle.loads(dump(includeCollectives=True, includeStackTraces=False, onlyActive=False))
        if not everything.get("entries"):
            return None
        active = pickle.loads(dump(includeCollectives=True, includeStackTraces=False, onlyActive=True))
        return len(active.get("entries", ()))
    except Exception:
        return None

# ... 65 lines not shown
        replay()
    e1.record()
    e1.synchronize()
    return e0.elapsed_time(e1) / n


class TrainStep:
    def __init__(self, model, optimizer, batch_size, window_size, horizon, units, series=None, world=1, graph=True,
                 exact=False, group=None, collective=None, one_graph=None, order_capacity=0, collective_fn=None,
                 schedule_check=None, attention_penalty=None, loss="mse", huber_delta=1.0, ignore_nan=False,
                 target_series=None):
        if loss not in _lib.SG_LOSS:
            raise ValueError(f"unknown loss {loss!r}: one of {sorted(_lib.SG_LOSS)}")
        self.loss_kw = {} if (loss == "mse" and not ignore_nan) else \
            dict(kind=loss, huber_delta=float(huber_delta), ignore_nan=bool(ignore_nan))
        if self.loss_kw and not hasattr(model, "loss"):
            raise ValueError("loss / ignore_nan need a model with the fused Model.loss")
        if target_series is not None and (series is None or target_series.shape != series.shape or
                                          target_series.device != series.device):
            raise ValueError("target_series must have the shape and device of `series`")
        self.target_series = target_series
        self.model, self.opt = model, optimizer
        self.collective_fn = collective_fn
        self.collective = (world > 1) if collective is None else bool(collective)
        if collective_fn is not None:
            self.collective = True
        self.one_graph = (os.environ.get("STEMGNN_DDP_ONE_GRAPH", "1") == "1") if one_graph is None else bool(one_graph)
        self.schedule_check = (os.environ.get("STEMGNN_SCHEDULE_CHECK", "1") != "0") if schedule_check is None \
            else bool(schedule_check)
        self.schedule = {"checked": False}
        if self.collective and self.one_graph and collective_fn is None:
            import torch.distributed as dist
            ok = dist.is_available() and dist.is_initialized() and dist.get_backend(group) == "nccl"
            self.one_graph = bool(ok)
        self.B, self.W, self.H, self.N = int(batch_size), int(window_size), int(horizon), int(units)
        self.world = world
        dev = next(model.parameters()).device
        self.device = dev
        self.fused = hasattr(optimizer, "bucket")
        self.bucket = optimizer.bucket if self.fused else (FlatGradBucket(model.parameters()) if self.collective else None)
        if self.bucket is not None:
            self.bucket.reduce_fn = collective_fn
        self.state = ops.set_direct_grad(model, self.fused, overlap=self.fused)
        self.fuse_zero = self.fused and getattr(optimizer, "fuse_zero_grad", False)
        self.series = series
        self.hi = torch.zeros(self.B, dtype=torch.int64, device=dev)
        if series is not None:
            self.hi.fill_(self.W)
        self.order = self.queue = None
        self._q_left = 0
        if series is not None and order_capacity > 0:
            self.order = torch.full((max(int(order_capacity), 4 * self.B),), self.W, dtype=torch.int64, device=dev)
            self.queue = torch.zeros(4, dtype=torch.int64, device=dev)
        self.x = torch.zeros(self.B, self.W, self.N, device=dev)
        self.y = torch.zeros(self.B, self.H, self.N, device=dev)
        self.loss = torch.zeros((), device=dev)
        self.loss_sum = torch.zeros((), device=dev, dtype=torch.float64)
        self._one = torch.ones((), device=dev)
        self.attention_penalty = attention_penalty
        self.penalty = torch.zeros((), device=dev) if attention_penalty is not None else None
        self.fuse_tail = hasattr(model, "loss")
        self.want_graph = bool(graph) and self.fused
        self.group = group
        if self.fused:
            self._grad_scale = 1.0 / world if self.collective else 1.0
        if exact and (world > 1 or self.collective):
            self.state.exact_group = (group, world, collective_fn)
            if not self.one_graph:
                self.want_graph = False
        self.mode = "eager"
        self._replay = None
        self._armed = False
        self._split = None
        self._tail_reduced = False
        if self.collective and self.fused and self.one_graph and self.state.overlap and hasattr(model, "stock_block"):
            self._split = self.bucket.offset_of(next(model.stock_block[0].parameters()))
            self.state.block_grads_hook = self._reduce_tail_range
        self._q_header = None
        if self.queue is not None:
            self._q_header = torch.zeros(4, dtype=torch.int64).pin_memory()

    def _fwd_bwd(self, hi, x, y):
        self._tail_reduced = False
        early = self.state.overlap and hasattr(self.model, "prefetch_side")
        if early:
            self.state.fork_event = torch.cuda.Event()
            self.state.fork_event.record()
        if self.series is not None:
            if hi is None:
                ops.window_gather_queue(self.series, self.order, self.queue, self.B, self.W, self.H, x, y, self.target_series)
            else:
                ops.window_gather(self.series, hi, self.W, self.H, x, y, self.target_series)
        if early:
            self.model.prefetch_side(self.device, batch=x.shape[0])
        if not self.fuse_zero:
            if self.bucket is not None:
                self.bucket.zero()
            else:
                self.model.zero_grad()
        attention = None
        if self.fuse_tail and self.attention_penalty is None:
            loss = self.model.loss(x, y, self.loss.detach(), self.loss_sum, unit_grad=True, **self.loss_kw)
        elif self.fuse_tail:
            loss, attention = self.model.loss(x, y, self.loss.detach(), self.loss_sum, unit_grad=True, return_attention=True,
                                              **self.loss_kw)
        else:
            forecast, attention = self.model(x)
            loss = ops.mse_loss(forecast, y, self.loss.detach(), self.loss_sum)
        if self.attention_penalty is None:
            torch.autograd.backward(loss, grad_tensors=(self._one,))
            return self.loss
        pen = self.attention_penalty(attention)
        if pen.shape != self._one.shape or pen.dtype != torch.float32 or pen.device != self._one.device:
            raise ValueError("attention_penalty must return a float32 scalar tensor on the model's device, got "
                             f"{pen.dtype} {tuple(pen.shape)} on {pen.device}")
        self.penalty.copy_(pen.detach())
        torch.autograd.backward([loss, pen], [self._one, self._one])
        return self.loss

    def _finish(self, loss):
        if not self.fused:
            self.opt.step()
            return
        prev, self.opt.grad_scale = self.opt.grad_scale, self._grad_scale
        try:
            self.opt.step()
        finally:
            self.opt.grad_scale = prev

    def _reduce_tail_range(self):
        self.bucket.all_reduce_range(self._split, self.bucket.numel, self.group, force=True)
        self._tail_reduced = True

    def _set_queue(self, position, count, wrap=0):
        h = self._q_header
        h[0], h[1], h[2], h[3] = int(position), 0, int(count), int(wrap)
        self.queue.copy_(h, non_blocking=False)

    def _all_ranks_ok(self, ok):
        import torch.distributed as dist
        if not (self.collective and dist.is_available() and dist.is_initialized()):
            return ok
        t = torch.tensor([1.0 if ok else 0.0], device=self.device)
        dist.all_reduce(t, op=dist.ReduceOp.MIN, group=self.group)
        return bool(t.item() > 0.5)

    def _sync(self):
        if self.collective:
            if self.fused and self._split is not None and self._tail_reduced:
                ops.join_side_streams(self.device)
                self.bucket.all_reduce_range(0, self._split, self.group, force=True)
            elif self.fused:
                if self._split is not None:
                    self.schedule["tail_hook_missed"] = self.schedule.get("tail_hook_missed", 0) + 1
                self.bucket.all_reduce_sum(self.group, force=True)
            else:
                self.bucket.all_reduce_mean(self.group)

    def _arm(self):
        if self.queue is None:
            return self._arm_inner()
        keep = self.queue.clone()
        self._set_queue(0, self.order.numel(), wrap=1)
        try:
            self._arm_inner()
        finally:
            self.queue.copy_(keep)

    def _whole(self):
        loss = self._fwd_bwd(None if self.queue is not None else self.hi, self.x, self.y)
        self._sync()
        self._finish(loss)

    def _arm_inner(self):
        self._armed = True
        if not self.want_graph:
            return
        if not self.collective or self.one_graph:
            snap = self._snapshot()
            rep = capture(self._whole, on_fail=self.state.reset)
            self.schedule["capture_drain"] = capture.last_drain
            self._restore(snap)
            if not self._all_ranks_ok(rep is not None):
                rep = None
            if rep is not None and self.collective and (self.world > 1 or self.collective_fn is not None):
                rep = self._verify_one_graph(rep)
            if rep is not None and self.schedule_check and self.state.overlap:
                rep = self._check_schedule(rep)
            if rep is None and self._split is not None:
                self._split, self.state.block_grads_hook = None, None
            if rep is not None:
                self._replay = rep
                self.mode = "hipgraph(whole step incl. rccl all-reduce)" if self.collective else "hipgraph(whole step)"
                if self.state.exact_group is not None:
                    self.mode = "hipgraph(whole step incl. the exact-mode attention collectives and the rccl all-reduce)"
                if self.schedule.get("side_branch_serialised"):
                    self.mode += " [side branch serialised: no branch overlap on this device]"
        if self._replay is None and self.collective and self.state.exact_group is None:
            box = {}

            def part_a():
# ... 363 lines not shown
```

### stemgnn_amd/ops.py

```python
import os
import weakref

import torch

from . import _lib

_NSPLIT = 32
_side_streams = {}


def _side_stream(device, index=0):
    key = (str(device), index)
    st = _side_streams.get(key)
    if st is None:
        st = torch.cuda.Stream(device=device)
        _side_streams[key] = st
    return st


def fresh_side_stream(device, index=0):
    _side_streams.pop((str(device), index), None)
    return _side_stream(device, index)


class HotPathState:

    def __init__(self):
        self.direct = False
        self.overlap = False
        self.prepacked = None
        self.preseed = None
        self.fork_event = None
        self.pending = None
        self.exact_group = None
        self.gru_front_live = False
        self.dh_factors = None
        self.block_grads_hook = None
        self.gru_ctl = None
        self.gru_ctl_zeroed = False
        self.warm_saved = None
        self.tail_finish = None
        self.side_probe = None
        _states.add(self)

    def set(self, direct=True, overlap=False):
        self.direct = bool(direct)
        self.overlap = bool(direct) and bool(overlap)
        return self

    def join(self):
        item, self.pending = self.pending, None
        if item is not None:
            side, keep = item
            torch.cuda.current_stream().wait_stream(side)
            del keep

    def reset(self):
        for item in (self.prepacked, self.pending):
            if item is not None:
                try:
                    (item[1] if item is self.prepacked else item[0]).synchronize()
                except RuntimeError:
                    pass
        self.prepacked = None
        self.preseed = None
        self.fork_event = None
        self.pending = None
        self.dh_factors = None
        self.gru_ctl_zeroed = False
        self.tail_finish = None


_states = weakref.WeakSet()
_NO_STATE = None


def _state(state):
    global _NO_STATE
    if state is not None:
        return state
    if _NO_STATE is None:
        _NO_STATE = HotPathState()
    return _NO_STATE


def join_side_streams(device=None):
    for st in list(_states):
        if st.pending is not None and (device is None or str(st.pending[0].device) == str(torch.device(device))):
            st.join()


def _all_reduce_mean(t, group_world):
    group, world = group_world[0], group_world[1]
    fn = group_world[2] if len(group_world) > 2 else None
    if fn is not None:
        fn(t)
    else:
        import torch.distributed as dist
        dist.all_reduce(t, op=dist.ReduceOp.SUM, group=group)
    t.div_(world)


def set_direct_grad(model, flag=True, overlap=False):
    return model.hot_state.set(flag, overlap)


_NCHUNK = 16


def _wg_cu(which, B, N):
    if which == 0:
        return 90
    if N > 512:
        return 50
    lib = _lib.load()
    cus = lib.stemgnn_num_cus()
    busy = lib.stemgnn_gru_bwd_cus(B, N)
    return max(10, min(100, (cus - busy) * 100 // cus))


def _stream():
    return torch.cuda.current_stream().cuda_stream


def glu_splits():
    v = os.environ.get("STEMGNN_DTYPE", "f32").lower()
    if v in ("f32", "fp32", ""):
        return 0
    if v == "bf16x3":
        return 3
    if v == "bf16x2":
        return 2
    raise _lib.StemGNNHipError(f"STEMGNN_DTYPE={v!r}: expected f32, bf16x3 or bf16x2")


def _pack_block(lib, parr, tables, pk, W, multi, splits, stream):
    if splits:
        _lib.check(lib.stemgnn_block_pack_panels(parr, tables.data_ptr(), pk.data_ptr(), W, multi, stream), "block_pack_panels")
    else:
        _lib.check(lib.stemgnn_block_pack(parr, tables.data_ptr(), pk.data_ptr(), W, multi, stream), "block_pack")


def _split_panels(lib, pk, W, multi, splits, device, stream):
    sp = torch.empty(lib.stemgnn_glu_split_floats(W, multi, splits), device=device, dtype=torch.float32)
    _lib.check(lib.stemgnn_glu_split_panels(pk.data_ptr(), sp.data_ptr(), W, multi, splits, stream), "glu_split_panels")
    return sp


def _require_gpu(t, name):
    if not t.is_cuda:
        raise _lib.StemGNNHipError(
            f"{name} is on {t.device}: stemgnn_amd runs only on a HIP device (no CPU fallback)")
    if t.dtype != torch.float32:
        raise _lib.StemGNNHipError(f"{name} must be float32, got {t.dtype}")


_table_cache = {}


def dft_tables(W, multi, device):
    key = (W, multi, str(device))
    t = _table_cache.get(key)
    if t is None:
        lib = _lib.load()
        n = lib.stemgnn_table_floats(W, multi)
        host = torch.empty(n, dtype=torch.float32)
        _lib.check(lib.stemgnn_make_tables_host(W, multi, host.data_ptr()), "make_tables_host")
        t = host.to(device)
        _table_cache[key] = t
    return t


def dropout_mask(drop_p, seed, B, N):
    lib = _lib.load()
    mask = torch.empty(B, N, N, device=seed.device, dtype=torch.float32)
    _lib.check(lib.stemgnn_dropout_mask(float(drop_p), seed.data_ptr(), B, N, mask.data_ptr(), _stream()),
               "dropout_mask")
    return mask


_gru_status = {}


def gru_status(device):
    key = str(device)
    t = _gru_status.get(key)
    if t is None:
        t = torch.zeros(1, dtype=torch.int32, device=device)
        _gru_status[key] = t
    return t


def gru_status_exists(device):
    return str(device) in _gru_status


def check_eigh_status(device=None):
    dev = torch.device(device) if device is not None else torch.device("cuda", torch.cuda.current_device())
    with torch.cuda.device(dev):
        rc = _lib.load().stemgnn_eigh_status()
    if rc == 2:
        raise _lib.StemGNNHipError(f"eigensolver status 2 on {dev}: a grid-barrier wait of the tridiagonalisation timed "
                                   "out (a workgroup of its cluster was not resident)")
    if rc == 3:
        raise _lib.StemGNNHipError(f"eigensolver status 3 on {dev}: the re-solve of an eigenvalue cluster broke down "
                                   "(no independent start vector left)")
    if rc != 0:
        raise _lib.StemGNNHipError(f"eigensolver status {rc} on {dev}")


def check_gru_status(device):
    st = gru_status(device)
    if int(st.item()) != 0:
        st.zero_()
        raise _lib.StemGNNHipError("GRU cluster exchange timed out (partner workgroup not resident?); "
                                   "set STEMGNN_GRU_CLUSTER=0 to use the single-workgroup kernels")


class GruFront(torch.autograd.Function):

    @staticmethod
    def forward(ctx, x, w_ih, w_hh, b_ih, b_hh, state=None):
        lib = _lib.load()
        ctx.state = _state(state)
        gru_params = (w_ih, w_hh, b_ih, b_hh)
        for name, t in (("x", x), ("GRU.weight_ih_l0", w_ih), ("GRU.weight_hh_l0", w_hh)):
            _require_gpu(t, name)
        x = x.contiguous()
        B, W, S = x.shape
        Hd = w_hh.shape[1]
        dev, f32 = x.device, torch.float32
        w_ih, w_hh, b_ih, b_hh = (t.contiguous() for t in (w_ih, w_hh, b_ih, b_hh))
        h_ext = torch.empty(S + 1, B, Hd, device=dev, dtype=f32)
        h_all = h_ext[1:]
        reserve = torch.empty(lib.stemgnn_gru_reserve_floats(B, S, Hd), device=dev, dtype=f32)
        scratch = torch.empty(lib.stemgnn_gru_fwd_scratch_floats(B, S, Hd), device=dev, dtype=f32)
        _lib.check(lib.stemgnn_gru_fwd(x.data_ptr(), w_ih.data_ptr(), w_hh.data_ptr(), b_ih.data_ptr(), b_hh.data_ptr(),
                                       B, S, Hd, W, scratch.data_ptr(), h_ext.data_ptr(), reserve.data_ptr(),
                                       gru_status(dev).data_ptr(), _stream()), "gru_fwd")
        ctx.save_for_backward(x, w_ih, w_hh, h_ext, reserve)
        ctx.gru_params = gru_params
        return h_all

    @staticmethod
    def backward(ctx, dh_all):
        lib = _lib.load()
        x, w_ih, w_hh, h_ext, reserve = ctx.saved_tensors
        B, W, S = x.shape
        Hd = w_hh.shape[1]
        dev, f32 = x.device, torch.float32
        factors, ctx.state.dh_factors = ctx.state.dh_factors, None
        if factors is None:
            dh_all = dh_all.contiguous()
        scratch = torch.empty(lib.stemgnn_gru_bwd_scratch_floats(B, S, Hd, W), device=dev, dtype=f32)
        prm = ctx.gru_params
        frozen = not any(ctx.needs_input_grad[1:5])
        direct = not frozen and ctx.state.direct and all(p.grad is not None and p.grad.is_contiguous() for p in prm)
        if direct:
            dw_ih, dw_hh, db_ih, db_hh = (p.grad for p in prm)
        elif not frozen:
            dw_ih, dw_hh = torch.empty_like(w_ih), torch.empty_like(w_hh)
            db_ih = torch.empty(3 * Hd, device=dev, dtype=f32)
            db_hh = torch.empty(3 * Hd, device=dev, dtype=f32)
        if frozen:
            if factors is not None:
                attn_scratch, fb, fn, wk, wq, after, dq_chunks = factors
                base = attn_scratch.data_ptr() + 4 * fn * fn
                ctx.state.gru_ctl_zeroed = False
                _lib.check(lib.stemgnn_gru_bwd_rank2_recur(base, base + 4 * fb * fn, dq_chunks, wk.data_ptr(), wq.data_ptr(),
                                                           x.data_ptr(), w_hh.data_ptr(), h_ext.data_ptr(), reserve.data_ptr(),
                                                           B, S, Hd, W, scratch.data_ptr(), gru_status(dev).data_ptr(),
                                                           _stream()), "gru_bwd_rank2_recur")
                if after is not None:
                    after()
            else:
                _lib.check(lib.stemgnn_gru_bwd_recur(dh_all.data_ptr(), x.data_ptr(), w_hh.data_ptr(), h_ext.data_ptr(),
                                                     reserve.data_ptr(), B, S, Hd, W, scratch.data_ptr(),
                                                     gru_status(dev).data_ptr(), _stream()), "gru_bwd_recur")
        elif factors is not None:
            attn_scratch, fb, fn, wk, wq, after, dq_chunks = factors
            base = attn_scratch.data_ptr() + 4 * fn * fn
            tail = (x.data_ptr(), w_hh.data_ptr(), h_ext.data_ptr(), reserve.data_ptr(), B, S, Hd, W, scratch.data_ptr(),
                    dw_ih.data_ptr(), dw_hh.data_ptr(), db_ih.data_ptr(), db_hh.data_ptr(), gru_status(dev).data_ptr())
            args = (base, base + 4 * fb * fn, wk.data_ptr(), wq.data_ptr()) + tail
            beside = (ctx.state.overlap and ctx.state.pending is not None and ctx.state.gru_ctl_zeroed
                      and bool(lib.stemgnn_gru_bwd_overlap_ok(B, S, Hd, W))
                      and ctx.state.gru_ctl.numel() == lib.stemgnn_gru_bwd_ctl_words(S))
            ctx.state.gru_ctl_zeroed = False
            ctl = ctx.state.gru_ctl.data_ptr() if beside else None
            if beside:
                _lib.check(lib.stemgnn_gru_bwd_rank2_begin(*args, ctl, _stream()), "gru_bwd_rank2_begin")
            elif dq_chunks:
                wg_split = 1 if glu_splits() == 2 and os.environ.get("STEMGNN_WGRAD_BF16", "1") != "0" else 0
                _lib.check(lib.stemgnn_gru_bwd_rank2_dq(base, base + 4 * fb * fn, dq_chunks, wg_split, wk.data_ptr(), wq.data_ptr(),
                                                        *tail, _stream()), "gru_bwd_rank2_dq")
            else:
                _lib.check(lib.stemgnn_gru_bwd_rank2(*args, _stream()), "gru_bwd_rank2")
            if after is not None:
                after()
            if beside:
                side = ctx.state.pending[0]
                _lib.check(lib.stemgnn_gru_bwd_rank2_finish(*args, ctl, side.cuda_stream, _stream()), "gru_bwd_rank2_finish")
        else:
            _lib.check(lib.stemgnn_gru_bwd(dh_all.data_ptr(), x.data_ptr(), w_hh.data_ptr(), h_ext.data_ptr(),
                                           reserve.data_ptr(), B, S, Hd, W, scratch.data_ptr(), dw_ih.data_ptr(),
                                           dw_hh.data_ptr(), db_ih.data_ptr(), db_hh.data_ptr(),
                                           gru_status(dev).data_ptr(), _stream()), "gru_bwd")
        dx = None
        if ctx.needs_input_grad[0]:
            dx = torch.empty(B, W, S, device=dev, dtype=f32)
            _lib.check(lib.stemgnn_gru_input_grad(scratch.data_ptr(), w_ih.data_ptr(), B, S, Hd, W, dx.data_ptr(), _stream()),
                       "gru_input_grad")
        ctx.state.join()
        if direct or frozen:
            return dx, None, None, None, None, None
        return dx, dw_ih, dw_hh, db_ih, db_hh, None


class FcTail(torch.autograd.Function):

    @staticmethod
    def forward(ctx, fsum, w0, b0, w2, b2, state=None):
# ... 182 lines not shown
        params = [None if p is None else p.contiguous() for p in params]
        tables = dft_tables(W, multi, dev)
        pk = torch.empty(lib.stemgnn_packed_floats(W, multi), device=dev, dtype=f32)
        sv = torch.empty(lib.stemgnn_saved_floats(B, N, W, multi), device=dev, dtype=f32)
        forecast = torch.empty(B, N, W, device=dev, dtype=f32)
        backcast = torch.empty(B, N, W, device=dev, dtype=f32) if has_bc else None
        parr = _lib.ptr_array(params)
        sb, sn, stt = N * W, W, 1
        _lib.check(lib.stemgnn_block_pack(parr, tables.data_ptr(), pk.data_ptr(), W, multi, st), "block_pack")
        _lib.check(lib.stemgnn_gft_fwd(mul_L.data_ptr(), X.data_ptr(), sb, sn, stt, sv.data_ptr(), B, N, W, st), "gft_fwd")
        _lib.check(lib.stemgnn_spectral_glu_fwd(pk.data_ptr(), sv.data_ptr(), B, N, W, multi, st), "spectral_glu_fwd")
        _lib.check(lib.stemgnn_igft_heads_fwd(parr, pk.data_ptr(), sv.data_ptr(), X.data_ptr(), sb, sn, stt,
                                              forecast.data_ptr(), 0, backcast.data_ptr() if has_bc else None,
                                              B, N, W, multi, st), "igft_heads_fwd")
        ctx.dims = (B, N, W, multi, bool(has_bc))
        ctx.params = params
        ctx.aux = (X, mul_L, tables, pk, sv, backcast.detach() if has_bc else None)
        if has_bc:
            return forecast, backcast
        return forecast, None

    @staticmethod
    def backward(ctx, dforecast, dbackcast):
        lib = _lib.load()
        B, N, W, multi, has_bc = ctx.dims
        X, mul_L, tables, pk, sv, backcast = ctx.aux
        params = ctx.params
        dev, f32 = X.device, torch.float32
        st = _stream()
        nsplit = _NSPLIT
        if dforecast is None:
            dforecast = torch.zeros(B, N, W, device=dev, dtype=f32)
        dforecast = dforecast.contiguous()
        use_bc = has_bc and dbackcast is not None
        if has_bc and not use_bc:
            dbackcast = torch.zeros(B, N, W, device=dev, dtype=f32)
            use_bc = True
        scratch = torch.empty(lib.stemgnn_scratch_floats(B, N, W, multi), device=dev, dtype=f32)
        dG = scratch[lib.stemgnn_scratch_offset_dG(B, N, W, multi):]
        gradpart = torch.empty(lib.stemgnn_gradpart_floats(W, multi, nsplit), device=dev, dtype=f32)
        dmul_L = torch.zeros(4, N, N, device=dev, dtype=f32)
        dX = torch.empty(B, N, W, device=dev, dtype=f32)
        parr = _lib.ptr_array(params)
        sb, sn, stt = N * W, W, 1
        _lib.check(lib.stemgnn_igft_heads_bwd(
            parr, pk.data_ptr(), sv.data_ptr(), X.data_ptr(), sb, sn, stt, dforecast.data_ptr(),
            dbackcast.contiguous().data_ptr() if use_bc else None, backcast.data_ptr() if use_bc else None,
            scratch.data_ptr(), gradpart.data_ptr(), nsplit, 1, B, N, W, multi, st), "igft_heads_bwd")
        _lib.check(lib.stemgnn_spectral_glu_bwd(pk.data_ptr(), sv.data_ptr(), scratch.data_ptr(), gradpart.data_ptr(),
                                                nsplit, 1, B, N, W, multi, st), "spectral_glu_bwd")
        _lib.check(lib.stemgnn_block_wgrad(parr, pk.data_ptr(), sv.data_ptr(), X.data_ptr(), sb, sn, stt,
                                           dforecast.data_ptr(), int(use_bc), scratch.data_ptr(), gradpart.data_ptr(),
                                           nsplit, 100, B, N, W, multi, st), "block_wgrad")
        _lib.check(lib.stemgnn_gft_bwd(mul_L.data_ptr(), X.data_ptr(), sb, sn, stt, dG.data_ptr(), dX.data_ptr(),
                                       dmul_L.data_ptr(), 0, B, N, W, st), "gft_bwd")
        grads = [None] * 33
        for i, p in enumerate(params):
            if p is None or (not has_bc and i in (7, 8)):
                continue
            grads[i] = torch.empty_like(p)
        _lib.check(lib.stemgnn_block_unpack_grads(gradpart.data_ptr(), nsplit, tables.data_ptr(), _lib.ptr_array(grads),
                                                  W, multi, int(has_bc), st), "block_unpack_grads")
        if use_bc and ctx.needs_input_grad[0]:
            _lib.check(lib.stemgnn_shortcut_dx(scratch.data_ptr(), params[7].data_ptr(), dX.data_ptr(), B, N, W, multi, st),
                       "shortcut_dx")
        return (dX, dmul_L, None, None, *grads)


_keep_attention_state = False
_last_attention_state = {}


def capture_attention_state(flag=True):
    global _keep_attention_state
    _keep_attention_state = bool(flag)
    if not flag:
        _last_attention_state.clear()


def last_attention_state(device):
    return _last_attention_state.get(str(torch.device(device)))


def prepack_blocks(state, block_params, W, multi, device, batch_shape=None):
    lib = _lib.load()
    side, main = _side_stream(device), torch.cuda.current_stream()
    tables = dft_tables(W, multi, device)
    n_packed = lib.stemgnn_packed_floats(W, multi)
    blocks = [[None if p is None else p.contiguous() for p in blk] for blk in block_params]
    packed = [torch.empty(n_packed, device=device, dtype=torch.float32) for _ in blocks]
    ev, state.fork_event = state.fork_event, None
    if ev is not None:
        side.wait_event(ev)
    else:
        side.wait_stream(main)
    splits = glu_splits()
    split = []
    for blk, pk in zip(blocks, packed):
        parr = _lib.ptr_array(blk)

        def pack(stream, parr=parr, pk=pk, blk=blk):
            _pack_block(lib, parr, tables, pk, W, multi, splits, stream)
        pack(side.cuda_stream)
        if state.side_probe is not None:
            state.side_probe.append(pack)
        if splits:
            split.append(_split_panels(lib, pk, W, multi, splits, device, side.cuda_stream))
    if batch_shape is not None and bool(lib.stemgnn_gru_bwd_overlap_ok(batch_shape[0], batch_shape[1], batch_shape[1], W)):
        nctl = lib.stemgnn_gru_bwd_ctl_words(batch_shape[1])
        if state.gru_ctl is None or state.gru_ctl.numel() != nctl or state.gru_ctl.device != torch.device(device):
            state.gru_ctl = torch.zeros(nctl, device=device, dtype=torch.int32)
        _lib.check(lib.stemgnn_fill_zero(state.gru_ctl.data_ptr(), 4 * nctl, side.cuda_stream), "fill_zero")
        state.gru_ctl_zeroed = True
    if batch_shape is not None and splits == 0 and os.environ.get("STEMGNN_GLU_WARM", "1") != "0":
        nwarm = lib.stemgnn_glu_warm_saved_floats(W, multi)
        if state.warm_saved is None or state.warm_saved.numel() != nwarm or state.warm_saved.device != torch.device(device):
            state.warm_saved = torch.zeros(nwarm, device=device, dtype=torch.float32)
        _lib.check(lib.stemgnn_spectral_glu_fwd_warm(packed[0].data_ptr(), split[0].data_ptr() if splits else None,
                                                     state.warm_saved.data_ptr(), batch_shape[0], batch_shape[1], W, multi,
                                                     splits, side.cuda_stream), "spectral_glu_fwd_warm")
    state.prepacked = (packed, side, blocks, (splits, split))


class SpectralHotPath(torch.autograd.Function):

    @staticmethod
    def forward(ctx, h, x, wk, wq, multi, alpha, drop_p, training, seed, state, *block_params):
        lib = _lib.load()
        state = ctx.state = _state(state)
        ctx.factored, state.gru_front_live = bool(getattr(state, "gru_front_live", False)), False
        for name, t in (("gru output", h), ("x", x), ("weight_key", wk), ("weight_query", wq)):
            _require_gpu(t, name)
        assert len(block_params) == 2 * _lib.SG_BLOCK_NPARAMS
        h = h.contiguous()
        x = x.contiguous()
        B, W, N = x.shape
        if h.shape != (N, B, N):
            raise _lib.StemGNNHipError(f"gru output must be [N,B,N]=({N},{B},{N}), got {tuple(h.shape)}")
        dev, f32 = x.device, torch.float32
        st = _stream()
        M = B * N
        blocks = [list(block_params[:33]), list(block_params[33:])]
        blocks = [[None if p is None else p.contiguous() for p in blk] for blk in blocks]
        tables = dft_tables(W, multi, dev)

        mul_L = torch.empty(4, N, N, device=dev, dtype=f32)
        attention = torch.empty(N, N, device=dev, dtype=f32)
        attn_saved = torch.empty(lib.stemgnn_attn_saved_floats(B, N), device=dev, dtype=f32)
        use_drop = bool(training) and drop_p > 0.0
        pre, state.prepacked = state.prepacked, None
        if pre is not None:
            torch.cuda.current_stream().wait_stream(pre[1])
        exact = state.exact_group
        for part in ((3,) if exact is None else (1, 2)):
            _lib.check(lib.stemgnn_attn_laplacian_fwd(
                h.data_ptr(), wk.data_ptr(), wq.data_ptr(), float(alpha), float(drop_p), int(bool(training)),
                seed.data_ptr() if use_drop else None, B, N, attn_saved.data_ptr(), attention.data_ptr(),
                mul_L.data_ptr(), part, st), "attn_laplacian_fwd")
            if exact is not None and part == 1:
                _all_reduce_mean(attn_saved[3 * B * N:3 * B * N + N * N + N], exact)
        if _keep_attention_state:
            _last_attention_state[str(dev)] = (attn_saved[:B * N].view(B, N).clone(),
                                               attn_saved[B * N:2 * B * N].view(B, N).clone())
        if os.environ.get("STEMGNN_SPECTRAL", "cheb") == "eig":
            lam = torch.empty(N, device=dev, dtype=f32)
            U = torch.empty(N, N, device=dev, dtype=f32)
            escr = torch.empty(lib.stemgnn_eigh_scratch_floats(N), device=dev, dtype=f32)
            _lib.check(lib.stemgnn_eigh_fwd(mul_L.data_ptr(), lam.data_ptr(), U.data_ptr(), escr.data_ptr(), N,
                                            0, st), "eigh_fwd")
        else:
            _lib.check(lib.stemgnn_cheb_fwd(mul_L.data_ptr(), N, st), "cheb_fwd")

        fsum = torch.empty(B, N, W, device=dev, dtype=f32)
        backcast = torch.empty(B, N, W, device=dev, dtype=f32)
        packed, saved, split = [], [], []
        splits = pre[3][0] if pre is not None else glu_splits()
        n_packed = lib.stemgnn_packed_floats(W, multi)
        n_saved = lib.stemgnn_saved_floats(B, N, W, multi)
        xviews = [(x, W * N, 1, N), (backcast, N * W, W, 1)]
        for s in range(2):
            sv = torch.empty(n_saved, device=dev, dtype=f32)
            parr = _lib.ptr_array(blocks[s])
            X, sb, sn, stt = xviews[s]
            sp = None
            if pre is not None:
                pk = pre[0][s]
                sp = pre[3][1][s] if splits else None
            else:
                pk = torch.empty(n_packed, device=dev, dtype=f32)
                _pack_block(lib, parr, tables, pk, W, multi, splits, st)
                if splits:
                    sp = _split_panels(lib, pk, W, multi, splits, dev, st)
            _lib.check(lib.stemgnn_gft_fwd(mul_L.data_ptr(), X.data_ptr(), sb, sn, stt, sv.data_ptr(), B, N, W, st),
                       "gft_fwd")
            if splits:
                _lib.check(lib.stemgnn_spectral_glu_fwd_split(pk.data_ptr(), sp.data_ptr(), sv.data_ptr(), B, N, W, multi,
                                                              splits, st), "spectral_glu_fwd_split")
            else:
                _lib.check(lib.stemgnn_spectral_glu_fwd(pk.data_ptr(), sv.data_ptr(), B, N, W, multi, st),
                           "spectral_glu_fwd")
            split.append(sp)
            _lib.check(lib.stemgnn_igft_heads_fwd(
                parr, pk.data_ptr(), sv.data_ptr(), X.data_ptr(), sb, sn, stt, fsum.data_ptr(), int(s == 1),
                backcast.data_ptr() if s == 0 else None, B, N, W, multi, st), "igft_heads_fwd")
            packed.append(pk)
            saved.append(sv)

        ctx.dims = (B, N, W, multi, float(alpha), float(drop_p), bool(training))
        ctx.blocks = blocks
        ctx.aux = (h, x, wk, wq, seed, tables, mul_L, attn_saved, backcast, packed, saved)
        ctx.split = (splits, split)
        ctx.mark_non_differentiable(mul_L)
        ctx.set_materialize_grads(False)
        return fsum, attention, mul_L

    @staticmethod
    def backward(ctx, dfsum, datt, _dmulL):
        if dfsum is None and datt is None:
            return (None,) * (10 + 2 * _lib.SG_BLOCK_NPARAMS)
        lib = _lib.load()
        B, N, W, multi, alpha, drop_p, training = ctx.dims
        h, x, wk, wq, seed, tables, mul_L, attn_saved, backcast, packed, saved = ctx.aux
        blocks = ctx.blocks
        state = ctx.state
        splits, split = ctx.split
        dev, f32 = x.device, torch.float32
        st = _stream()
        tail_finish, state.tail_finish = state.tail_finish, None
        if dfsum is None and tail_finish is not None:
            dfsum = torch.zeros(B, N, W, device=dev, dtype=f32)
        attn_only = dfsum is None
        if not attn_only:
            dfsum = dfsum.contiguous()
        if datt is not None:
            datt = datt.contiguous()
        nsplit = _NSPLIT
        n_scratch = lib.stemgnn_scratch_floats(B, N, W, multi)
        off_dG = lib.stemgnn_scratch_offset_dG(B, N, W, multi)
        n_gradpart = lib.stemgnn_gradpart_floats(W, multi, nsplit)
        dmul_L = None if attn_only else torch.empty(4, N, N, device=dev, dtype=f32)
        dbackcast = None if attn_only else torch.empty(B, N, W, device=dev, dtype=f32)
        xviews = [(x, W * N, 1, N), (backcast, N * W, W, 1)]
        grads = [[None] * 33, [None] * 33]
        direct_idx = set()
        nig = ctx.needs_input_grad
        live = [not attn_only and any(nig[10 + 33 * s + i] for i, p in enumerate(blocks[s]) if p is not None) for s in (0, 1)]
        kq_live = nig[2] or nig[3]
        for s in (1, 0):
            for i, p in enumerate(blocks[s]):
                if p is None or (s == 1 and i in (7, 8)) or not live[s]:
                    continue
                if state.direct and p.grad is not None and p.grad.is_contiguous():
                    grads[s][i] = p.grad
                    direct_idx.add((s, i))
                else:
                    grads[s][i] = torch.empty_like(p)
        n_block_grads = sum(g is not None for blk in grads for g in blk)
        overlap = state.overlap and n_block_grads > 0 and len(direct_idx) == n_block_grads
        side = _side_stream(dev) if overlap else None
        main = torch.cuda.current_stream()
        keep = []
        if tail_finish is not None and not overlap:
# ... 235 lines not shown
    w0, b0, w2, b2 = (t.contiguous() for t in fc_params)
    H = w2.shape[0]
    forecast = torch.empty(B, H, N, device=dev, dtype=f32)
    _lib.check(lib.stemgnn_fc_tail_fwd(fsum.data_ptr(), w0.data_ptr(), b0.data_ptr(), w2.data_ptr(), b2.data_ptr(),
                                       B, N, W, H, forecast.data_ptr(), st), "fc_tail_fwd")
    return forecast, attention


def forecast_store(forecast, target, pos, out_forecast, out_target):
    lib = _lib.load()
    B, H, N = forecast.shape
    if target.shape != forecast.shape or out_forecast.shape[1:] != (H, N) or out_target.shape != out_forecast.shape:
        raise _lib.StemGNNHipError("forecast_store: shape mismatch")
    if pos.dtype != torch.int64 or pos.device != forecast.device:
        raise _lib.StemGNNHipError("forecast_store: pos must be an int64 tensor on the forecast's device")
    _lib.check(lib.stemgnn_forecast_store(forecast.data_ptr(), target.data_ptr(), pos.data_ptr(), out_forecast.data_ptr(),
                                          out_target.data_ptr(), B, H, N, out_forecast.shape[0], _stream()), "forecast_store")


class MSELossFn(torch.autograd.Function):

    @staticmethod
    def forward(ctx, forecast, target, loss_out=None, accum=None):
        lib = _lib.load()
        _require_gpu(forecast, "forecast")
        _require_gpu(target, "target")
        if forecast.shape != target.shape:
            raise _lib.StemGNNHipError(f"MSE: shapes differ {tuple(forecast.shape)} vs {tuple(target.shape)}")
        forecast, target = forecast.contiguous(), target.contiguous()
        scratch = torch.empty(lib.stemgnn_mse_scratch_floats(), device=forecast.device, dtype=torch.float32)
        loss = loss_out if loss_out is not None else torch.empty((), device=forecast.device, dtype=torch.float32)
        if accum is not None and (accum.dtype != torch.float64 or accum.device != forecast.device):
            raise _lib.StemGNNHipError("MSE: accum must be a float64 scalar on the forecast's device")
        _lib.check(lib.stemgnn_mse_fwd(forecast.data_ptr(), target.data_ptr(), forecast.numel(), scratch.data_ptr(),
                                       loss.data_ptr(), accum.data_ptr() if accum is not None else None, _stream()),
                   "mse_fwd")
        ctx.save_for_backward(forecast, target)
        ctx.set_materialize_grads(False)
        if loss_out is not None:
            ctx.mark_dirty(loss_out)
        return loss

    @staticmethod
    def backward(ctx, grad_loss):
        lib = _lib.load()
        forecast, target = ctx.saved_tensors
        grad_loss = grad_loss.contiguous()
        dforecast = torch.empty_like(forecast)
        _lib.check(lib.stemgnn_mse_bwd(forecast.data_ptr(), target.data_ptr(), forecast.numel(), grad_loss.data_ptr(),
                                       dforecast.data_ptr(), _stream()), "mse_bwd")
        return dforecast, None, None, None


def mse_loss(forecast, target, loss_out=None, accum=None):
    return MSELossFn.apply(forecast, target, loss_out, accum)


class MSELoss(torch.nn.Module):

    def __init__(self, reduction="mean"):
        super().__init__()
        if reduction != "mean":
            raise ValueError("stemgnn_amd.ops.MSELoss implements reduction='mean' only (the reference's setting)")

    def forward(self, forecast, target):
        return MSELossFn.apply(forecast, target)


def normalize_series(raw, sub, div, clip01):
    lib = _lib.load()
    if not raw.is_cuda or raw.dtype != torch.float64:
        raise _lib.StemGNNHipError("normalize_series: raw must be a float64 tensor on a HIP device")
    raw, sub, div = raw.contiguous(), sub.contiguous(), div.contiguous()
    T, N = raw.shape
    out = torch.empty(T, N, device=raw.device, dtype=torch.float32)
    _lib.check(lib.stemgnn_normalize_series(raw.data_ptr(), sub.data_ptr(), div.data_ptr(), int(bool(clip01)),
                                            out.data_ptr(), T, N, _stream()), "normalize_series")
    return out


_gather_status = {}


def _check_target_series(series, target_series, what):
    _require_gpu(target_series, "target_series")
    if target_series.shape != series.shape or target_series.device != series.device or not target_series.is_contiguous():
        raise _lib.StemGNNHipError(f"{what}: target_series must be a contiguous [T,N] tensor of the series' shape and device")


def window_gather(series, hi, W, H, x=None, y=None, target_series=None):
    lib = _lib.load()
    _require_gpu(series, "series")
    if hi.dtype != torch.int64 or hi.device != series.device:
        raise _lib.StemGNNHipError("window_gather: hi must be an int64 tensor on the series' device")
    T, N = series.shape
    B = hi.numel()
    if x is None:
        x = torch.empty(B, W, N, device=series.device, dtype=torch.float32)
    if y is None:
        y = torch.empty(B, H, N, device=series.device, dtype=torch.float32)
    key = str(series.device)
    st = _gather_status.get(key)
    if st is None:
        st = _gather_status[key] = torch.zeros(1, dtype=torch.int32, device=series.device)
    if target_series is not None:
        _check_target_series(series, target_series, "window_gather")
        _lib.check(lib.stemgnn_window_gather_pair(series.data_ptr(), target_series.data_ptr(), hi.data_ptr(), x.data_ptr(),
                                                  y.data_ptr(), B, W, H, N, T, st.data_ptr(), _stream()), "window_gather")
        return x, y
    _lib.check(lib.stemgnn_window_gather(series.data_ptr(), hi.data_ptr(), x.data_ptr(), y.data_ptr(), B, W, H, N, T,
                                         st.data_ptr(), _stream()), "window_gather")
    return x, y


def window_gather_queue(series, order, queue, B, W, H, x, y, target_series=None):
    lib = _lib.load()
    _require_gpu(series, "series")
    for t, n in ((order, "order"), (queue, "queue")):
        if t.dtype != torch.int64 or t.device != series.device or not t.is_contiguous():
            raise _lib.StemGNNHipError(f"window_gather_queue: {n} must be a contiguous int64 tensor on the series' device")
    T, N = series.shape
    key = str(series.device)
    st = _gather_status.get(key)
    if st is None:
        st = _gather_status[key] = torch.zeros(1, dtype=torch.int32, device=series.device)
    if target_series is not None:
        _check_target_series(series, target_series, "window_gather_queue")
        _lib.check(lib.stemgnn_window_gather_queue_pair(series.data_ptr(), target_series.data_ptr(), order.data_ptr(),
                                                        queue.data_ptr(), x.data_ptr(), y.data_ptr(), B, W, H, N, T,
                                                        st.data_ptr(), _stream()), "window_gather_queue")
        return x, y
    _lib.check(lib.stemgnn_window_gather_queue(series.data_ptr(), order.data_ptr(), queue.data_ptr(), x.data_ptr(),
                                               y.data_ptr(), B, W, H, N, T, st.data_ptr(), _stream()), "window_gather_queue")
    return x, y


def check_gather_status(device):
    st = _gather_status.get(str(device))
    if st is not None:
        v = int(st.item())
        if v != 0:
            st.zero_()
            raise IndexError("window_gather: window index outside the series" if v & 1 else
                             "window_gather_queue: stepped past the end of the loaded order")


def roll_window(inputs, forecast, forecast_steps, step, horizon):
    lib = _lib.load()
    _require_gpu(inputs, "inputs")
    _require_gpu(forecast, "forecast")
    B, W, N = inputs.shape
    L = forecast.shape[1]
    if L == 0:
        raise Exception("Get blank inference result")
    inputs, forecast = inputs.contiguous(), forecast.contiguous()
    nxt = torch.empty_like(inputs)
    _lib.check(lib.stemgnn_roll_window(inputs.data_ptr(), forecast.data_ptr(), nxt.data_ptr(),
                                       forecast_steps.data_ptr(), B, W, L, N, int(step), int(horizon), _stream()),
               "roll_window")
    return nxt


def eval_metrics(target, forecast, mul=None, add=None, ignore_nan=False):
    lib = _lib.load()
    _require_gpu(target, "target")
    _require_gpu(forecast, "forecast")
# ... 17 lines not shown
```

Measured before the change: 85580.

## Fuse window gather into GRU input-projection kernel and pack all blocks in one launch

Folds the training-window gather (copying series rows into x/y from a device-side order queue) into the GRU gi_stream kernel. Extra workgroups write x/y while the main workgroups read windows straight from the series, and the queue is advanced by the last workgroup. Block weight packing for both spectral blocks, plus the dropout seed advance, moves into a single launch. The goal is fewer kernel launches and less host overhead in the per-step prologue, at the cost of added atomics, extra workgroups and more complex control flow.

```diff
diff --git a/include/stemgnn_hip.h b/include/stemgnn_hip.h
--- a/include/stemgnn_hip.h
+++ b/include/stemgnn_hip.h
@@ -96,6 +96,11 @@
 int stemgnn_gru_fwd(const float* x, const float* w_ih, const float* w_hh, const float* b_ih, const float* b_hh,
                     int B, int S, int Hd, int W, float* scratch, float* h_ext, float* reserve, int* status,
                     void* stream);
+int stemgnn_gru_fwd_gather(const float* series_x, const float* series_y, const long long* order, long long* queue, float* x,
+                           float* y, int H, long T, int* gather_status, const float* w_ih, const float* w_hh,
+                           const float* b_ih, const float* b_hh, int B, int S, int Hd, int W, float* scratch, float* h_ext,
+                           float* reserve, int* status, void* stream);
+int stemgnn_gru_fwd_gather_fused(int B, int S, int Hd, int W);
 int stemgnn_gru_bwd(const float* dh_all, const float* x, const float* w_hh, const float* h_ext,
                     const float* reserve, int B, int S, int Hd, int W, float* scratch,
                     float* dw_ih, float* dw_hh, float* db_ih, float* db_hh, int* status, void* stream);
@@ -133,6 +138,8 @@
 int stemgnn_block_pack_panels(const float* const* params_host, const float* tables, float* packed, int W, int multi,
                               void* stream);
 int stemgnn_glu_fused_repack(float* packed, int W, int multi, void* stream);
+int stemgnn_blocks_pack_all(const float* const* params_host, int nblocks, const float* tables, float* const* packed, int W,
+                            int multi, uint64_t* seed, uint64_t* used, void* stream);
 int stemgnn_block_unpack_grads(const float* gradpart, int nsplit, const float* tables,
                                float* const* grads_host, int W, int multi, int has_backcast, void* stream);
 
diff --git a/stemgnn_amd/_lib.py b/stemgnn_amd/_lib.py
--- a/stemgnn_amd/_lib.py
+++ b/stemgnn_amd/_lib.py
@@ -68,6 +68,9 @@
     "stemgnn_gru_bwd_cus": (c_int, [c_int, c_int]),
     "stemgnn_gru_paths": (c_int, [c_int, c_int, c_int, c_int, c_int, POINTER(c_int)]),
     "stemgnn_gru_fwd": (c_int, [_P, _P, _P, _P, _P, c_int, c_int, c_int, c_int, _P, _P, _P, _P, _P]),
+    "stemgnn_gru_fwd_gather": (c_int, [_P, _P, _P, _P, _P, _P, c_int, c_long, _P, _P, _P, _P, _P,
+                                       c_int, c_int, c_int, c_int, _P, _P, _P, _P, _P]),
+    "stemgnn_gru_fwd_gather_fused": (c_int, [c_int, c_int, c_int, c_int]),
     "stemgnn_gru_bwd": (c_int, [_P, _P, _P, _P, _P, c_int, c_int, c_int, c_int, _P, _P, _P, _P, _P, _P, _P]),
     "stemgnn_gru_bwd_rank2_ok": (c_int, [c_int, c_int]),
     "stemgnn_gru_bwd_rank2": (c_int, [_P, _P, _P, _P, _P, _P, _P, _P, c_int, c_int, c_int, c_int, _P, _P, _P, _P, _P, _P, _P]),
@@ -112,6 +115,7 @@
     "stemgnn_eval_metrics_masked": (c_int, [_P, _P, _P, _P, c_long, c_int, c_int, _P, _P, _P]),
     "stemgnn_block_pack": (c_int, [_PP, _P, _P, c_int, c_int, _P]),
     "stemgnn_block_pack_panels": (c_int, [_PP, _P, _P, c_int, c_int, _P]),
+    "stemgnn_blocks_pack_all": (c_int, [_PP, c_int, _P, _PP, c_int, c_int, _P, _P, _P]),
     "stemgnn_block_unpack_grads": (c_int, [_P, c_int, _P, _PP, c_int, c_int, c_int, _P]),
     "stemgnn_gft_fwd": (c_int, [_P, _P, c_long, c_long, c_long, _P, c_int, c_int, c_int, _P]),
     "stemgnn_gft_bwd": (c_int, [_P, _P, c_long, c_long, c_long, _P, _P, _P, c_int, c_int, c_int, c_int, _P]),
diff --git a/stemgnn_amd/base_model.py b/stemgnn_amd/base_model.py
--- a/stemgnn_amd/base_model.py
+++ b/stemgnn_amd/base_model.py
@@ -89,7 +89,7 @@
         self.hot_state = ops.HotPathState()
         self.to(device)
 
-    def _next_seed(self, device):
+    def _dropout_key(self, device):
         if self._seed is None or self._seed.device != device:
             rank = 0
             if torch.distributed.is_available() and torch.distributed.is_initialized():
@@ -98,7 +98,10 @@
                                                  else torch.cuda.current_device()].initial_seed()
                    + 0x9E3779B97F4A7C15 * (self._instance + 1) + 0xD1B54A32D192ED03 * rank) % (1 << 62)
             self._seed = torch.tensor([key, 0], dtype=torch.int64, device=device)
-        used = torch.empty_like(self._seed)
+        return self._seed
+
+    def _next_seed(self, device):
+        used = torch.empty_like(self._dropout_key(device))
         _lib.check(_lib.load().stemgnn_dropout_seed_next(self._seed.data_ptr(), used.data_ptr(),
                                                          torch.cuda.current_stream(device).cuda_stream), "dropout_seed_next")
         return used
@@ -134,9 +137,13 @@
             return
         device = device or self.weight_key.device
         blocks = (self.stock_block[0].hip_params(), self.stock_block[1].hip_params())
-        ops.prepack_blocks(hs, blocks, self.time_step, self.multi_layer, device,
-                           batch_shape=None if batch is None else (int(batch), self.unit))
-        if self.training and self.dropout_rate > 0.0:
+        use_drop = self.training and self.dropout_rate > 0.0
+        used = ops.prepack_blocks(hs, blocks, self.time_step, self.multi_layer, device,
+                                  batch_shape=None if batch is None else (int(batch), self.unit),
+                                  dropout_key=self._dropout_key(device) if use_drop and ops.pack_is_one_launch() else None)
+        if used is not None:
+            hs.preseed = used
+        elif use_drop:
             with torch.cuda.stream(ops._side_stream(device)):
                 hs.preseed = self._next_seed(device)
 
@@ -152,17 +159,23 @@
         blocks = (self.stock_block[0].hip_params(), self.stock_block[1].hip_params())
         use_drop = self.training and self.dropout_rate > 0.0
         hs = self.hot_state
-        if hs.overlap and hs.prepacked is None:
+        miopen = os.environ.get("STEMGNN_GRU", "hip") == "miopen"
+        if miopen:
+            ops.flush_pending_gather(hs)
+        side_late = hs.pending_gather is not None
+        if hs.overlap and hs.prepacked is None and not side_late:
             self.prefetch_side(x.device, batch=x.shape[0])
-        seed, hs.preseed = hs.preseed, None
-        if seed is not None and not torch.cuda.is_current_stream_capturing():
-            seed.record_stream(torch.cuda.current_stream())
-        if os.environ.get("STEMGNN_GRU", "hip") == "miopen":
+        if miopen:
             h, _ = self.GRU(x.permute(2, 0, 1).contiguous())
         else:
             g = self.GRU
             h = GruFront.apply(x, g.weight_ih_l0, g.weight_hh_l0, g.bias_ih_l0, g.bias_hh_l0, hs)
             hs.gru_front_live = True
+        if hs.overlap and hs.prepacked is None and side_late:
+            self.prefetch_side(x.device, batch=x.shape[0])
+        seed, hs.preseed = hs.preseed, None
+        if seed is not None and not torch.cuda.is_current_stream_capturing():
+            seed.record_stream(torch.cuda.current_stream())
         if use_drop and seed is None:
             seed = self._next_seed(x.device)
         params = blocks[0] + blocks[1]
diff --git a/stemgnn_amd/csrc/glu_fused.h b/stemgnn_amd/csrc/glu_fused.h
--- a/stemgnn_amd/csrc/glu_fused.h
+++ b/stemgnn_amd/csrc/glu_fused.h
@@ -31,9 +31,13 @@
   int K[3], np[2][3], cp[2][3];
   GfGeom g;
 };
-static __global__ __launch_bounds__(256) void sg_pack_fused_kernel(const GfPackArgs a) {
-  const int r = blockIdx.y;
-  const size_t e = (size_t)blockIdx.x * 256 + threadIdx.x;
+struct GfPanelRead {
+  const float* const (*wp)[3];
+  const int (*np)[3];
+  __device__ __forceinline__ float operator()(int r, int l, int k, int q) const { return wp[r][l][(size_t)k * np[r][l] + q]; }
+};
+template <class Src>
+__device__ __forceinline__ void gf_pack_elem(const GfPackArgs& a, int r, size_t e, const Src& src, float* __restrict__ wf) {
   if (e >= (size_t)a.g.ns * GF_STAGE) return;
   int s = (int)(e / GF_STAGE), l = 0;
   while (l < 2 && s >= a.g.nst[l]) { s -= a.g.nst[l]; ++l; }
@@ -43,8 +47,11 @@
   const int wave = p / (64 * hp), rem = p % (64 * hp), h = rem >> 6, fi = (rem & 63) >> 1, t = rem & 1;
   const int c = wave * 32 * hp + h * 32 + fi, k = s * a.g.rs[l] + kk;
   float v = 0.f;
-  if (k < a.K[l] && c < a.cp[r][l]) v = a.wp[r][l][(size_t)k * a.np[r][l] + ((c >> 4) << 5) + (c & 15) + 16 * t];
-  a.wf[r][e] = v;
+  if (k < a.K[l] && c < a.cp[r][l]) v = src(r, l, k, ((c >> 4) << 5) + (c & 15) + 16 * t);
+  wf[e] = v;
+}
+static __global__ __launch_bounds__(256) void sg_pack_fused_kernel(const GfPackArgs a) {
+  gf_pack_elem(a, blockIdx.y, (size_t)blockIdx.x * 256 + threadIdx.x, GfPanelRead{a.wp, a.np}, a.wf[blockIdx.y]);
 }
 
 struct GfArgs {
@@ -274,9 +281,8 @@
   int CP, KG;
   GdGeom g;
 };
-static __global__ __launch_bounds__(256) void sg_pack_dgrad_kernel(const GdPackArgs a) {
-  const int r = blockIdx.y;
-  const size_t e = (size_t)blockIdx.x * 256 + threadIdx.x;
+template <class Src>
+__device__ __forceinline__ void gd_pack_elem(const GdPackArgs& a, int r, size_t e, const Src& src, float* __restrict__ wd) {
   if (e >= (size_t)a.g.ns[r] * GF_STAGE) return;
   int s = (int)(e / GF_STAGE);
   const int nt = a.g.nt, rs = a.g.rs, nc = 128 * nt;
@@ -291,8 +297,8 @@
     const int t = k2 & 1, wf = k2 >> 1, w2 = wf >> 5, f2 = wf & 31;
     const int c2 = w2 * 32 * nt + 32 * ph + f2;
     float v = 0.f;
-    if (w2 < 4 && c2 < a.CP && kin < a.KG) v = a.wp[r][0][(size_t)kin * a.np[r][0] + ((c2 >> 4) << 5) + (c2 & 15) + 16 * t];
-    a.wd[r][e] = v;
+    if (w2 < 4 && c2 < a.CP && kin < a.KG) v = src(r, 0, kin, ((c2 >> 4) << 5) + (c2 & 15) + 16 * t);
+    wd[e] = v;
     return;
   }
   const int kk = wi / nc, p = wi % nc;
@@ -303,7 +309,7 @@
   float v = 0.f;
   if (s < a.g.nstA[r]) {
     const int q = s * rs + kk;
-    if (q < a.np[r][2] && c < a.CP) v = a.wp[r][2][(size_t)c * a.np[r][2] + q];
+    if (q < a.np[r][2] && c < a.CP) v = src(r, 2, c, q);
   } else {
     s -= a.g.nstA[r];
     int ph = 0;
@@ -311,9 +317,12 @@
     const int k2 = s * rs + kk;
     const int t = k2 & 1, wf = k2 >> 1, w2 = wf >> 5, f2 = wf & 31;
     const int c2 = w2 * 32 * nt + 32 * ph + f2;
-    if (w2 < 4 && c2 < a.CP && c < a.CP) v = a.wp[r][1][(size_t)c * a.np[r][1] + ((c2 >> 4) << 5) + (c2 & 15) + 16 * t];
-  }
-  a.wd[r][e] = v;
+    if (w2 < 4 && c2 < a.CP && c < a.CP) v = src(r, 1, c, ((c2 >> 4) << 5) + (c2 & 15) + 16 * t);
+  }
+  wd[e] = v;
+}
+static __global__ __launch_bounds__(256) void sg_pack_dgrad_kernel(const GdPackArgs a) {
+  gd_pack_elem(a, blockIdx.y, (size_t)blockIdx.x * 256 + threadIdx.x, GfPanelRead{a.wp, a.np}, a.wd[blockIdx.y]);
 }
 
 struct GdArgs {
diff --git a/stemgnn_amd/csrc/gru.hip b/stemgnn_amd/csrc/gru.hip
--- a/stemgnn_amd/csrc/gru.hip
+++ b/stemgnn_amd/csrc/gru.hip
@@ -61,15 +61,80 @@
   }
 };
 
+struct GruGatherArgs {
+  const float *series_x, *series_y;
+  const long long* order;
+  long long* q;
+  float *x, *y;
+  int* gstatus;
+  long T;
+  int H, nrb, nextra;
+};
+struct GruWindow { long long h0; bool have, ok; };
+template <int W>
+__device__ __forceinline__ GruWindow gru_window(const GruGatherArgs& ga, long long pos, long long count, int b) {
+  GruWindow w;
+  w.have = pos >= 0 && pos + b < count;
+  w.h0 = w.have ? ga.order[pos + b] : 0;
+  w.ok = w.have && w.h0 - W >= 0 && w.h0 + ga.H <= ga.T;
+  return w;
+}
+__device__ __forceinline__ void gru_queue_advance(const GruGatherArgs& ga, long long ticket, long long pos, long long count,
+                                                  int B) {
+  if (ticket != (long long)gridDim.x * gridDim.y - 1) return;
+  __hip_atomic_store(&ga.q[1], 0ll, __ATOMIC_RELAXED, __HIP_MEMORY_SCOPE_AGENT);
+  long long next = pos + B;
+  if (ga.q[3] != 0 && next + B > count) next = 0;
+  __hip_atomic_store(&ga.q[0], next, __ATOMIC_RELAXED, __HIP_MEMORY_SCOPE_AGENT);
+}
+__device__ __forceinline__ void gru_gi_zero_share(unsigned* __restrict__ za, unsigned* __restrict__ zb, unsigned na, unsigned nb) {
+  if (na + nb) {
+    const unsigned nwg = gridDim.x * gridDim.y, id = blockIdx.y * gridDim.x + blockIdx.x;
+    const unsigned per = (na + nb + nwg - 1) / nwg, hi = min(na + nb, (id + 1) * per);
+    for (unsigned i = id * per + threadIdx.x; i < hi; i += blockDim.x) {
+      if (i < na) za[i] = 0u;
+      else zb[i - na] = 0u;
+    }
+  }
+}
 constexpr int GI_RB = 16, GI_NT = 192;
-template <int W>
+template <int W, bool GQ>
 __global__ __launch_bounds__(GI_NT) void gru_gi_stream_kernel(const float* __restrict__ x, const float* __restrict__ w_ih,
                                                               const float* __restrict__ b_ih, float* __restrict__ gi, int B,
                                                               int S, int Hd, unsigned* __restrict__ za,
-                                                              unsigned* __restrict__ zb, unsigned na, unsigned nb) {
+                                                              unsigned* __restrict__ zb, unsigned na, unsigned nb,
+                                                              const GruGatherArgs ga) {
   __shared__ float xs[GI_RB][W];
   const int tid = threadIdx.x;
   const int M = S * B, H3 = 3 * Hd, ncg = H3 >> 2;
+  long long pos = 0, count = 0;
+  if (GQ) {
+    pos = __hip_atomic_load(&ga.q[0], __ATOMIC_RELAXED, __HIP_MEMORY_SCOPE_AGENT);
+    count = ga.q[2];
+    if ((int)blockIdx.x >= ga.nrb) {
+      const int e = blockIdx.y * ga.nextra + ((int)blockIdx.x - ga.nrb), E = ga.nextra * gridDim.y;
+      const int R = W + ga.H, n4 = S >> 2;
+      const size_t total = (size_t)R * B * n4;
+      for (size_t idx = (size_t)e * GI_NT + tid; idx < total; idx += (size_t)E * GI_NT) {
+        const int row = (int)(idx / n4), i4 = (int)(idx - (size_t)row * n4);
+        const int b = row / R, r = row - b * R;
+        const GruWindow w = gru_window<W>(ga, pos, count, b);
+        float* dst = r < W ? ga.x + ((size_t)b * W + r) * S : ga.y + ((size_t)b * ga.H + (r - W)) * S;
+        const float* src = (r < W ? ga.series_x : ga.series_y) + (size_t)(w.ok ? w.h0 - W + r : 0) * S;
+        reinterpret_cast<float4*>(dst)[i4] = w.ok ? reinterpret_cast<const float4*>(src)[i4] : make_float4(0.f, 0.f, 0.f, 0.f);
+      }
+      if (e == 0 && ga.gstatus)
+        for (int b = tid; b < B; b += GI_NT) {
+          const GruWindow w = gru_window<W>(ga, pos, count, b);
+          if (!w.ok) atomicOr(ga.gstatus, w.have ? 1 : 2);
+        }
+      gru_gi_zero_share(za, zb, na, nb);
+      __syncthreads();
+      if (tid == 0)
+        gru_queue_advance(ga, __hip_atomic_fetch_add(&ga.q[1], 1ll, __ATOMIC_RELAXED, __HIP_MEMORY_SCOPE_AGENT), pos, count, B);
+      return;
+    }
+  }
   const int i0 = blockIdx.x * GI_RB;
   const int cg = blockIdx.y * GI_NT + tid;
   const bool live = cg < ncg;
@@ -94,17 +159,17 @@
     const int r = e / W, k = e - r * W;
     const int i = i0 + r < M ? i0 + r : M - 1;
     const int sI = i / B, b = i - sI * B;
-    xs[r][k] = x[((size_t)b * W + k) * S + sI];
-  }
-  if (na + nb) {
-    const unsigned nwg = gridDim.x * gridDim.y, id = blockIdx.y * gridDim.x + blockIdx.x;
-    const unsigned per = (na + nb + nwg - 1) / nwg, hi = min(na + nb, (id + 1) * per);
-    for (unsigned i = id * per + tid; i < hi; i += GI_NT) {
-      if (i < na) za[i] = 0u;
-      else zb[i - na] = 0u;
-    }
-  }
+    if (GQ) {
+      const GruWindow w = gru_window<W>(ga, pos, count, b);
+      xs[r][k] = w.ok ? ga.series_x[(size_t)(w.h0 - W + k) * S + sI] : 0.f;
+    } else {
+      xs[r][k] = x[((size_t)b * W + k) * S + sI];
+    }
+  }
+  gru_gi_zero_share(za, zb, na, nb);
   __syncthreads();
+  long long ticket = -1;
+  if (GQ && tid == 0) ticket = __hip_atomic_fetch_add(&ga.q[1], 1ll, __ATOMIC_RELAXED, __HIP_MEMORY_SCOPE_AGENT);
 #pragma unroll 4
   for (int r = 0; r < GI_RB; ++r) {
     float a0 = 0.f, a1 = 0.f, a2 = 0.f, a3 = 0.f;
@@ -119,6 +184,7 @@
     if (live && i0 + r < M)
       *reinterpret_cast<float4*>(gi + (size_t)(i0 + r) * H3 + 4 * cg) = make_float4(a0 + bias.x, a1 + bias.y, a2 + bias.z, a3 + bias.w);
   }
+  if (GQ && tid == 0) gru_queue_advance(ga, ticket, pos, count, B);
 }
 
 __global__ void gru_transpose_kernel(const float* __restrict__ w, float* __restrict__ wT, int rows, int cols) {
@@ -946,14 +1012,23 @@
   return B * (pl.P > 0 ? pl.P : 1);
 }
 
+static bool gru_gather_fused(const GruPlan& pl, int S) { return pl.gi_stream && (S & 3) == 0; }
 template <bool RS>
 static int gru_fwd_impl(const float* x, const float* w_ih, const float* w_hh, const float* b_ih, const float* b_hh, int B,
-                        int S, int Hd, int W, float* scratch, float* h_ext, float* reserve, int* status, void* stream) {
+                        int S, int Hd, int W, float* scratch, float* h_ext, float* reserve, int* status, void* stream,
+                        const GruGatherArgs* gq = nullptr) {
   if (!x || !w_ih || !w_hh || !b_ih || !b_hh || !scratch || !h_ext || (RS && !reserve) || !status || B <= 0 || S <= 0 ||
       Hd <= 0 || W <= 0)
     return SG_EINVAL;
   hipStream_t st = (hipStream_t)stream;
   const GruPlan pl = gru_plan(B, S, Hd, W, gru_resident_limit());
+  const bool gi16 = (reinterpret_cast<uintptr_t>(scratch + (size_t)3 * Hd * Hd) & 15) == 0;
+  const bool fuse_gather = gq && gru_gather_fused(pl, S) && gi16;
+  if (gq && !fuse_gather) {
+    const int rc = stemgnn_window_gather_queue_pair(gq->series_x, gq->series_y, gq->order, gq->q, gq->x, gq->y, B, W, gq->H,
+                                                    S, gq->T, gq->gstatus, stream);
+    if (rc) return rc;
+  }
   const bool use_wide = pl.fwd_family == SG_GRU_FAM_WIDE, use_c4 = pl.fwd_family == SG_GRU_FAM_CLUSTER4;
   float* h_all = h_ext + (size_t)B * Hd;
   float* w_hhT = scratch;
@@ -965,11 +1040,22 @@
   } else {
     SG_TRY(sg_zero_async(h_ext, (size_t)B * Hd * sizeof(float), st));
   }
-  if (pl.gi_stream && (reinterpret_cast<uintptr_t>(gi) & 15) == 0) {
+  if (fuse_gather) {
+    const int ncg = 3 * Hd / 4, nrb = (S * B + GI_RB - 1) / GI_RB;
+    const size_t total4 = (size_t)(W + gq->H) * B * (S >> 2);
+    GruGatherArgs ga = *gq;
+    ga.nrb = nrb;
+    ga.nextra = (int)((total4 + (size_t)GI_NT * 4 - 1) / ((size_t)GI_NT * 4));
+    ga.nextra = ga.nextra < 1 ? 1 : (ga.nextra > 64 ? 64 : ga.nextra);
+    hipLaunchKernelGGL((gru_gi_stream_kernel<12, true>), dim3(nrb + ga.nextra, (ncg + GI_NT - 1) / GI_NT), dim3(GI_NT), 0,
+                       st, x, w_ih, b_ih, gi, B, S, Hd, reinterpret_cast<unsigned*>(h_ext), reinterpret_cast<unsigned*>(xbuf2),
+                       (unsigned)zn0, (unsigned)zn1, ga);
+    SG_TRY(hipGetLastError());
+  } else if (pl.gi_stream && (reinterpret_cast<uintptr_t>(gi) & 15) == 0) {
     const int ncg = 3 * Hd / 4;
-    hipLaunchKernelGGL(gru_gi_stream_kernel<12>, dim3((S * B + GI_RB - 1) / GI_RB, (ncg + GI_NT - 1) / GI_NT), dim3(GI_NT), 0,
+    hipLaunchKernelGGL((gru_gi_stream_kernel<12, false>), dim3((S * B + GI_RB - 1) / GI_RB, (ncg + GI_NT - 1) / GI_NT), dim3(GI_NT), 0,
                        st, x, w_ih, b_ih, gi, B, S, Hd, reinterpret_cast<unsigned*>(h_ext), reinterpret_cast<unsigned*>(xbuf2),
-                       (unsigned)zn0, (unsigned)zn1);
+                       (unsigned)zn0, (unsigned)zn1, GruGatherArgs{});
     SG_TRY(hipGetLastError());
   } else {
     GruGiOp op{x, w_ih, b_ih, gi, B, S, Hd, W, reinterpret_cast<unsigned*>(h_ext), reinterpret_cast<unsigned*>(xbuf2),
@@ -1026,6 +1112,22 @@
                                const float* b_hh, int B, int S, int Hd, int W, float* scratch, float* h_ext,
                                float* reserve, int* status, void* stream) {
   return gru_fwd_impl<true>(x, w_ih, w_hh, b_ih, b_hh, B, S, Hd, W, scratch, h_ext, reserve, status, stream);
+}
+extern "C" int stemgnn_gru_fwd_gather(const float* series_x, const float* series_y, const long long* order, long long* queue,
+                                      float* x, float* y, int H, long T, int* gather_status, const float* w_ih,
+                                      const float* w_hh, const float* b_ih, const float* b_hh, int B, int S, int Hd, int W,
+                                      float* scratch, float* h_ext, float* reserve, int* status, void* stream) {
+  if (!series_x || !series_y || !order || !queue || !x || !y || B <= 0 || W <= 0 || H < 0 || S <= 0 || T < (long)W + H)
+    return SG_EINVAL;
+  if ((S & 3) == 0 && ((((uintptr_t)series_x | (uintptr_t)series_y | (uintptr_t)x | (uintptr_t)y) & 15) != 0)) return SG_EINVAL;
+  GruGatherArgs ga{series_x, series_y, order, queue, x, y, gather_status, T, H, 0, 0};
+  return gru_fwd_impl<true>(x, w_ih, w_hh, b_ih, b_hh, B, S, Hd, W, scratch, h_ext, reserve, status, stream, &ga);
+}
+extern "C" int stemgnn_gru_fwd_gather_fused(int B, int S, int Hd, int W) {
+  if (B <= 0 || S <= 0 || Hd <= 0 || W <= 0) return 0;
+  int limit = gru_resident_limit();
+  if (limit <= 0) limit = gru_limit_of_cus(256);
+  return gru_gather_fused(gru_plan(B, S, Hd, W, limit), S) ? 1 : 0;
 }
 extern "C" int stemgnn_gru_fwd_infer(const float* x, const float* w_ih, const float* w_hh, const float* b_ih,
                                      const float* b_hh, int B, int S, int Hd, int W, float* scratch, float* h_ext,
diff --git a/stemgnn_amd/csrc/pack.hip b/stemgnn_amd/csrc/pack.hip
--- a/stemgnn_amd/csrc/pack.hip
+++ b/stemgnn_amd/csrc/pack.hip
@@ -71,11 +71,39 @@
   return sg_grad_layout(sg_dims(1, 1, W, multi), nsplit).total;
 }
 
-__global__ void sg_pack_kernel(SgBlockParams prm, const float* __restrict__ tab, float* __restrict__ packed, SgDims d,
-                               SgPackedLayout P, SgTableLayout T) {
-  const size_t idx = (size_t)blockIdx.x * blockDim.x + threadIdx.x;
+__device__ __forceinline__ float sg_panel_weight(const SgBlockParams& prm, const float* __restrict__ tab, const SgDims& d,
+                                                 const SgTableLayout& T, int r, int l, int kk, int q) {
+  const int W = d.W, C = d.C, cu = sg_glu_cu(d, l, r), g = 2 * l + r;
+  const int c = ((q >> 5) << 4) + (q & 15), side = (q >> 4) & 1;
+  float val = 0.f;
+  if (c < cu) {
+    const int ch = l < 2 ? c : sg_l2_orig_channel(d, r, c);
+    const float* w = prm.p[sg_pidx_glu(g, side, 0)];
+    if (l == 0) {
+      const int kq = kk / W + 1, t = kk - (kq - 1) * W;
+      const float* row = w + (size_t)ch * (4 * W) + kq * W;
+      const float* dt = tab + (r ? T.sinW : T.cosW) + t * W;
+      float s = 0.f;
+      for (int f = 0; f < W; ++f) s = fmaf(dt[f], row[f], s);
+      val = r ? -s : s;
+    } else if (kk < C) {
+      val = w[(size_t)ch * C + kk];
+    }
+  }
+  return val;
+}
+struct SgPanelCalc {
+  const SgBlockParams& prm;
+  const float* tab;
+  const SgDims& d;
+  const SgTableLayout& T;
+  __device__ __forceinline__ float operator()(int r, int l, int k, int q) const { return sg_panel_weight(prm, tab, d, T, r, l, k, q); }
+};
+
+__device__ __forceinline__ void sg_pack_panels_elem(const SgBlockParams& prm, const float* __restrict__ tab, float* __restrict__ packed,
+                                                    const SgDims& d, const SgPackedLayout& P, const SgTableLayout& T, size_t idx) {
   if (idx >= P.total) return;
-  const int W = d.W, Wm = d.Wm, C = d.C;
+  const int Wm = d.Wm;
   float val = 0.f;
   if (idx >= P.wfold) {
     const size_t e = idx - P.wfold;
@@ -107,22 +135,7 @@
       if (idx >= P.w[r][l] && idx < P.w[r][l] + (size_t)kin * np) {
         const size_t e = idx - P.w[r][l];
         const int kk = (int)(e / np), q = (int)(e - (size_t)kk * np);
-        const int c = ((q >> 5) << 4) + (q & 15), side = (q >> 4) & 1;
-        if (c < cu) {
-          const int ch = l < 2 ? c : sg_l2_orig_channel(d, r, c);
-          const float* w = prm.p[sg_pidx_glu(g, side, 0)];
-          if (l == 0) {
-            const int kq = kk / W + 1, t = kk - (kq - 1) * W;
-            const float* row = w + (size_t)ch * (4 * W) + kq * W;
-            const float* dt = tab + (r ? T.sinW : T.cosW) + t * W;
-            float s = 0.f;
-            for (int f = 0; f < W; ++f) s = fmaf(dt[f], row[f], s);
-            val = r ? -s : s;
-          } else if (kk < C) {
-            val = w[(size_t)ch * C + kk];
-          }
-        }
-        packed[idx] = val;
+        packed[idx] = sg_panel_weight(prm, tab, d, T, r, l, kk, q);
         return;
       }
       if (idx >= P.b[r][l] && idx < P.b[r][l] + (size_t)np) {
@@ -136,6 +149,10 @@
         return;
       }
     }
+}
+__global__ void sg_pack_kernel(SgBlockParams prm, const float* __restrict__ tab, float* __restrict__ packed, SgDims d,
+                               SgPackedLayout P, SgTableLayout T) {
+  sg_pack_panels_elem(prm, tab, packed, d, P, T, (size_t)blockIdx.x * blockDim.x + threadIdx.x);
 }
 
 extern "C" int stemgnn_block_pack_panels(const float* const* params_host, const float* tables, float* packed, int W,
@@ -160,41 +177,127 @@
   return stemgnn_glu_fused_repack(packed, W, multi, stream);
 }
 
+static GfPackArgs sg_gf_pack_args(const SgDims& d, const SgPackedLayout& P, const GfGeom& gg, float* packed) {
+  GfPackArgs a;
+  a.g = gg;
+  for (int l = 0; l < 3; ++l) {
+    a.K[l] = sg_glu_kin(d, l);
+    for (int r = 0; r < 2; ++r) {
+      a.wp[r][l] = packed ? packed + P.w[r][l] : nullptr;
+      a.np[r][l] = sg_glu_np(d, l, r);
+      a.cp[r][l] = sg_glu_cp(d, l, r);
+    }
+  }
+  for (int r = 0; r < 2; ++r) a.wf[r] = packed ? packed + P.wfused[r] : nullptr;
+  return a;
+}
+static GdPackArgs sg_gd_pack_args(const SgDims& d, const SgPackedLayout& P, const GdGeom& gd, float* packed) {
+  GdPackArgs a;
+  a.g = gd;
+  a.CP = d.CP; a.KG = d.KG;
+  for (int l = 0; l < 3; ++l)
+    for (int r = 0; r < 2; ++r) {
+      a.wp[r][l] = packed ? packed + P.w[r][l] : nullptr;
+      a.np[r][l] = sg_glu_np(d, l, r);
+    }
+  for (int r = 0; r < 2; ++r) a.wd[r] = packed ? packed + P.wdgrad[r] : nullptr;
+  return a;
+}
+static unsigned sg_gf_pack_wgs(const GfGeom& gg) { return (unsigned)(((size_t)gg.ns * GF_STAGE + 255) / 256); }
+static unsigned sg_gd_pack_wgs(const GdGeom& gd) {
+  const int nsmax = gd.ns[0] > gd.ns[1] ? gd.ns[0] : gd.ns[1];
+  return (unsigned)(((size_t)nsmax * GF_STAGE + 255) / 256);
+}
 extern "C" int stemgnn_glu_fused_repack(float* packed, int W, int multi, void* stream) {
   if (!packed || W <= 0 || multi <= 0) return SG_EINVAL;
   const SgDims d = sg_dims(1, 1, W, multi);
   const SgPackedLayout P = sg_packed_layout(d);
   const GfGeom gg = gf_geom(d);
   if (gg.ok) {
-    GfPackArgs a;
-    a.g = gg;
-    for (int l = 0; l < 3; ++l) {
-      a.K[l] = sg_glu_kin(d, l);
-      for (int r = 0; r < 2; ++r) {
-        a.wp[r][l] = packed + P.w[r][l];
-        a.np[r][l] = sg_glu_np(d, l, r);
-        a.cp[r][l] = sg_glu_cp(d, l, r);
-      }
-    }
-    for (int r = 0; r < 2; ++r) a.wf[r] = packed + P.wfused[r];
-    const unsigned fb = (unsigned)(((size_t)gg.ns * GF_STAGE + 255) / 256);
-    hipLaunchKernelGGL(sg_pack_fused_kernel, dim3(fb, 2), dim3(256), 0, (hipStream_t)stream, a);
+    hipLaunchKernelGGL(sg_pack_fused_kernel, dim3(sg_gf_pack_wgs(gg), 2), dim3(256), 0, (hipStream_t)stream,
+                       sg_gf_pack_args(d, P, gg, packed));
     SG_TRY(hipGetLastError());
   }
   const GdGeom gd = gd_geom(d);
   if (gd.ok) {
-    GdPackArgs a;
-    a.g = gd;
-    a.CP = d.CP; a.KG = d.KG;
-    for (int l = 0; l < 3; ++l)
-      for (int r = 0; r < 2; ++r) {
-        a.wp[r][l] = packed + P.w[r][l];
-        a.np[r][l] = sg_glu_np(d, l, r);
-      }
-    for (int r = 0; r < 2; ++r) a.wd[r] = packed + P.wdgrad[r];
-    const int nsmax = gd.ns[0] > gd.ns[1] ? gd.ns[0] : gd.ns[1];
-    const unsigned fb = (unsigned)(((size_t)nsmax * GF_STAGE + 255) / 256);
-    hipLaunchKernelGGL(sg_pack_dgrad_kernel, dim3(fb, 2), dim3(256), 0, (hipStream_t)stream, a);
+    hipLaunchKernelGGL(sg_pack_dgrad_kernel, dim3(sg_gd_pack_wgs(gd), 2), dim3(256), 0, (hipStream_t)stream,
+                       sg_gd_pack_args(d, P, gd, packed));
+    SG_TRY(hipGetLastError());
+  }
+  return 0;
+}
+
+constexpr int SG_PACK_ALL_MAXB = 2;
+struct SgPackAllArgs {
+  SgBlockParams prm[SG_PACK_ALL_MAXB];
+  float* packed[SG_PACK_ALL_MAXB];
+  const float* tab;
+  SgDims d;
+  SgPackedLayout P;
+  SgTableLayout T;
+  GfPackArgs gf;
+  GdPackArgs gd;
+  unsigned nA, nF, nD;
+  uint64_t *seed, *used;
+};
+__global__ __launch_bounds__(256) void sg_pack_all_kernel(const SgPackAllArgs a) {
+  const int blk = blockIdx.y;
+  unsigned x = blockIdx.x;
+  if (a.seed && blk == 0 && x == 0 && threadIdx.x == 0) {
+    const uint64_t key = a.seed[0], off = a.seed[1];
+    a.used[0] = key;
+    a.used[1] = off;
+    a.seed[1] = off + 1;
+  }
+  const SgBlockParams& prm = a.prm[blk];
+  float* packed = a.packed[blk];
+  if (x < a.nA) {
+    sg_pack_panels_elem(prm, a.tab, packed, a.d, a.P, a.T, (size_t)x * 256 + threadIdx.x);
+    return;
+  }
+  x -= a.nA;
+  const SgPanelCalc src{prm, a.tab, a.d, a.T};
+  if (x < 2 * a.nF) {
+    const int r = x >= a.nF;
+    gf_pack_elem(a.gf, r, (size_t)(x - r * a.nF) * 256 + threadIdx.x, src, packed + a.P.wfused[r]);
+    return;
+  }
+  x -= 2 * a.nF;
+  const int r = x >= a.nD;
+  gd_pack_elem(a.gd, r, (size_t)(x - r * a.nD) * 256 + threadIdx.x, src, packed + a.P.wdgrad[r]);
+}
+
+extern "C" int stemgnn_blocks_pack_all(const float* const* params_host, int nblocks, const float* tables, float* const* packed,
+                                       int W, int multi, uint64_t* seed, uint64_t* used, void* stream) {
+  if (!params_host || !tables || !packed || nblocks <= 0 || W <= 0 || multi <= 0) return SG_EINVAL;
+  if ((seed == nullptr) != (used == nullptr) || (seed && seed == used)) return SG_EINVAL;
+  for (int b = 0; b < nblocks; ++b) {
+    if (!packed[b]) return SG_EINVAL;
+    for (int i = 0; i < SG_BLOCK_NPARAMS; ++i)
+      if (!params_host[(size_t)b * SG_BLOCK_NPARAMS + i] && i != 5 && i != 6) return SG_EINVAL;
+  }
+  SgPackAllArgs a;
+  a.tab = tables;
+  a.d = sg_dims(1, 1, W, multi);
+  a.P = sg_packed_layout(a.d);
+  a.T = sg_table_layout(a.d);
+  const GfGeom gg = gf_geom(a.d);
+  const GdGeom gd = gd_geom(a.d);
+  a.gf = sg_gf_pack_args(a.d, a.P, gg, nullptr);
+  a.gd = sg_gd_pack_args(a.d, a.P, gd, nullptr);
+  a.nA = (unsigned)((a.P.total + 255) / 256);
+  a.nF = gg.ok ? sg_gf_pack_wgs(gg) : 0;
+  a.nD = gd.ok ? sg_gd_pack_wgs(gd) : 0;
+  for (int b0 = 0; b0 < nblocks; b0 += SG_PACK_ALL_MAXB) {
+    const int nb = nblocks - b0 < SG_PACK_ALL_MAXB ? nblocks - b0 : SG_PACK_ALL_MAXB;
+    for (int b = 0; b < nb; ++b) {
+      for (int i = 0; i < SG_BLOCK_NPARAMS; ++i) a.prm[b].p[i] = params_host[(size_t)(b0 + b) * SG_BLOCK_NPARAMS + i];
+      a.packed[b] = packed[b0 + b];
+    }
+    for (int b = nb; b < SG_PACK_ALL_MAXB; ++b) { a.prm[b] = a.prm[0]; a.packed[b] = a.packed[0]; }
+    a.seed = b0 == 0 ? seed : nullptr;
+    a.used = b0 == 0 ? used : nullptr;
+    hipLaunchKernelGGL(sg_pack_all_kernel, dim3(a.nA + 2 * a.nF + 2 * a.nD, nb), dim3(256), 0, (hipStream_t)stream, a);
     SG_TRY(hipGetLastError());
   }
   return 0;
diff --git a/stemgnn_amd/engine.py b/stemgnn_amd/engine.py
--- a/stemgnn_amd/engine.py
+++ b/stemgnn_amd/engine.py
@@ -171,16 +171,23 @@
 
     def _fwd_bwd(self, hi, x, y):
         self._tail_reduced = False
+        self.state.pending_gather = None
         early = self.state.overlap and hasattr(self.model, "prefetch_side")
         if early:
             self.state.fork_event = torch.cuda.Event()
             self.state.fork_event.record()
+        handed = False
         if self.series is not None:
-            if hi is None:
+            if hi is None and self._gather_in_front(x):
+                ops.check_gather_operands(self.series, self.order, self.queue, self.target_series)
+                self.state.pending_gather = (self.series, self.order, self.queue, self.B, self.W, self.H, x, y,
+                                             self.target_series)
+                handed = True
+            elif hi is None:
                 ops.window_gather_queue(self.series, self.order, self.queue, self.B, self.W, self.H, x, y, self.target_series)
             else:
                 ops.window_gather(self.series, hi, self.W, self.H, x, y, self.target_series)
-        if early:
+        if early and not handed:
             self.model.prefetch_side(self.device, batch=x.shape[0])
         if not self.fuse_zero:
             if self.bucket is not None:
@@ -196,6 +203,9 @@
         else:
             forecast, attention = self.model(x)
             loss = ops.mse_loss(forecast, y, self.loss.detach(), self.loss_sum)
+        if self.state.pending_gather is not None:
+            self.state.pending_gather = None
+            raise RuntimeError("TrainStep: the forward did not run the window gather it was handed")
         if self.attention_penalty is None:
             torch.autograd.backward(loss, grad_tensors=(self._one,))
             return self.loss
@@ -206,6 +216,15 @@
         self.penalty.copy_(pen.detach())
         torch.autograd.backward([loss, pen], [self._one, self._one])
         return self.loss
+
+    def _gather_in_front(self, x):
+        m = self.model
+        if not ops.prologue_fused() or os.environ.get("STEMGNN_GRU", "hip") == "miopen" or x.requires_grad:
+            return False
+        if getattr(m, "hot_state", None) is not self.state or not hasattr(m, "GRU"):
+            return False
+        B, W, N = x.shape
+        return bool(_lib.load().stemgnn_gru_fwd_gather_fused(B, N, m.GRU.hidden_size, W))
 
     def _finish(self, loss):
         if not self.fused:
diff --git a/stemgnn_amd/ops.py b/stemgnn_amd/ops.py
--- a/stemgnn_amd/ops.py
+++ b/stemgnn_amd/ops.py
@@ -1,3 +1,4 @@
+import ctypes
 import os
 import weakref
 
@@ -41,6 +42,7 @@
         self.warm_saved = None
         self.tail_finish = None
         self.side_probe = None
+        self.pending_gather = None
         _states.add(self)
 
     def set(self, direct=True, overlap=False):
@@ -69,6 +71,7 @@
         self.dh_factors = None
         self.gru_ctl_zeroed = False
         self.tail_finish = None
+        self.pending_gather = None
 
 
 _states = weakref.WeakSet()
@@ -123,6 +126,20 @@
     return torch.cuda.current_stream().cuda_stream
 
 
+def prologue_fused():
+    return os.environ.get("STEMGNN_PROLOGUE_FUSED", "1") != "0"
+
+
+def pack_is_one_launch():
+    return glu_splits() == 0 and prologue_fused()
+
+
+def flush_pending_gather(state):
+    pg, state.pending_gather = state.pending_gather, None
+    if pg is not None:
+        window_gather_queue(*pg)
+
+
 def glu_splits():
     v = os.environ.get("STEMGNN_DTYPE", "f32").lower()
     if v in ("f32", "fp32", ""):
@@ -139,6 +156,20 @@
         _lib.check(lib.stemgnn_block_pack_panels(parr, tables.data_ptr(), pk.data_ptr(), W, multi, stream), "block_pack_panels")
     else:
         _lib.check(lib.stemgnn_block_pack(parr, tables.data_ptr(), pk.data_ptr(), W, multi, stream), "block_pack")
+
+
+def _pack_all_thunk(lib, blocks, tables, packed, W, multi):
+    parr = (ctypes.c_void_p * (_lib.SG_BLOCK_NPARAMS * len(blocks)))()
+    for i, blk in enumerate(blocks):
+        for j, t in enumerate(blk):
+            parr[i * _lib.SG_BLOCK_NPARAMS + j] = None if t is None else t.data_ptr()
+    pkarr = (ctypes.c_void_p * len(packed))(*(pk.data_ptr() for pk in packed))
+
+    def pack_all(stream, key=None, _keep=(blocks, packed, tables)):
+        _lib.check(lib.stemgnn_blocks_pack_all(parr, len(blocks), tables.data_ptr(), pkarr, W, multi,
+                                               None if key is None else key[0].data_ptr(),
+                                               None if key is None else key[1].data_ptr(), stream), "blocks_pack_all")
+    return pack_all
 
 
 def _split_panels(lib, pk, W, multi, splits, device, stream):
@@ -235,9 +266,24 @@
         h_all = h_ext[1:]
         reserve = torch.empty(lib.stemgnn_gru_reserve_floats(B, S, Hd), device=dev, dtype=f32)
         scratch = torch.empty(lib.stemgnn_gru_fwd_scratch_floats(B, S, Hd), device=dev, dtype=f32)
-        _lib.check(lib.stemgnn_gru_fwd(x.data_ptr(), w_ih.data_ptr(), w_hh.data_ptr(), b_ih.data_ptr(), b_hh.data_ptr(),
-                                       B, S, Hd, W, scratch.data_ptr(), h_ext.data_ptr(), reserve.data_ptr(),
-                                       gru_status(dev).data_ptr(), _stream()), "gru_fwd")
+        pg = ctx.state.pending_gather
+        if pg is not None and (pg[6].data_ptr() != x.data_ptr() or tuple(pg[6].shape) != (B, W, S) or pg[3] != B):
+            flush_pending_gather(ctx.state)
+            pg = None
+        if pg is not None:
+            ctx.state.pending_gather = None
+            series, order, queue, _, _, H, _, y, target = pg
+            tgt = series if target is None else target
+            _lib.check(lib.stemgnn_gru_fwd_gather(series.data_ptr(), tgt.data_ptr(), order.data_ptr(), queue.data_ptr(),
+                                                  x.data_ptr(), y.data_ptr(), H, series.shape[0],
+                                                  gather_status(dev).data_ptr(), w_ih.data_ptr(), w_hh.data_ptr(),
+                                                  b_ih.data_ptr(), b_hh.data_ptr(), B, S, Hd, W, scratch.data_ptr(),
+                                                  h_ext.data_ptr(), reserve.data_ptr(), gru_status(dev).data_ptr(),
+                                                  _stream()), "gru_fwd_gather")
+        else:
+            _lib.check(lib.stemgnn_gru_fwd(x.data_ptr(), w_ih.data_ptr(), w_hh.data_ptr(), b_ih.data_ptr(), b_hh.data_ptr(),
+                                           B, S, Hd, W, scratch.data_ptr(), h_ext.data_ptr(), reserve.data_ptr(),
+                                           gru_status(dev).data_ptr(), _stream()), "gru_fwd")
         ctx.save_for_backward(x, w_ih, w_hh, h_ext, reserve)
         ctx.gru_params = gru_params
         return h_all
@@ -586,7 +632,7 @@
     return _last_attention_state.get(str(torch.device(device)))
 
 
-def prepack_blocks(state, block_params, W, multi, device, batch_shape=None):
+def prepack_blocks(state, block_params, W, multi, device, batch_shape=None, dropout_key=None):
     lib = _lib.load()
     side, main = _side_stream(device), torch.cuda.current_stream()
     tables = dft_tables(W, multi, device)
@@ -600,7 +646,19 @@
         side.wait_stream(main)
     splits = glu_splits()
     split = []
+    used = None
+    one_launch = pack_is_one_launch()
+    if one_launch:
+        pack_all = _pack_all_thunk(lib, blocks, tables, packed, W, multi)
+        if dropout_key is not None:
+            with torch.cuda.stream(side):
+                used = torch.empty_like(dropout_key)
+        pack_all(side.cuda_stream, None if used is None else (dropout_key, used))
+        if state.side_probe is not None:
+            state.side_probe.append(pack_all)
     for blk, pk in zip(blocks, packed):
+        if one_launch:
+            break
         parr = _lib.ptr_array(blk)
 
         def pack(stream, parr=parr, pk=pk, blk=blk):
@@ -624,6 +682,7 @@
                                                      state.warm_saved.data_ptr(), batch_shape[0], batch_shape[1], W, multi,
                                                      splits, side.cuda_stream), "spectral_glu_fwd_warm")
     state.prepacked = (packed, side, blocks, (splits, split))
+    return used
 
 
 class SpectralHotPath(torch.autograd.Function):
@@ -682,6 +741,9 @@
         n_packed = lib.stemgnn_packed_floats(W, multi)
         n_saved = lib.stemgnn_saved_floats(B, N, W, multi)
         xviews = [(x, W * N, 1, N), (backcast, N * W, W, 1)]
+        if pre is None and pack_is_one_launch():
+            pre = ([torch.empty(n_packed, device=dev, dtype=f32) for _ in range(2)], None, None, (0, []))
+            _pack_all_thunk(lib, blocks, tables, pre[0], W, multi)(st)
         for s in range(2):
             sv = torch.empty(n_saved, device=dev, dtype=f32)
             parr = _lib.ptr_array(blocks[s])
@@ -1083,6 +1145,23 @@
 _gather_status = {}
 
 
+def gather_status(device):
+    key = str(device)
+    st = _gather_status.get(key)
+    if st is None:
+        st = _gather_status[key] = torch.zeros(1, dtype=torch.int32, device=device)
+    return st
+
+
+def check_gather_operands(series, order, queue, target_series=None):
+    _require_gpu(series, "series")
+    for t, n in ((order, "order"), (queue, "queue")):
+        if t.dtype != torch.int64 or t.device != series.device or not t.is_contiguous():
+            raise _lib.StemGNNHipError(f"window_gather_queue: {n} must be a contiguous int64 tensor on the series' device")
+    if target_series is not None:
+        _check_target_series(series, target_series, "window_gather_queue")
+
+
 def _check_target_series(series, target_series, what):
     _require_gpu(target_series, "target_series")
     if target_series.shape != series.shape or target_series.device != series.device or not target_series.is_contiguous():
```

Measured after the change: 85590, median of 2. About the same (+0.0%).
